# linomp/INF560-approximate-pattern-matching

Hardware: AMD Instinct MI355X
Metric: window-DP-cells/sec (higher is better)
Workload: dtype u32

## Files before the change

inf560-approximate-pattern-matching_amd/csrc/apm_device.h:

```cpp
#ifndef APM_DEVICE_H
#define APM_DEVICE_H

#include "apm_internal.h"
#include "apm_core.h"

__device__ __forceinline__ uint32_t apm_wave_count(bool pred) {
    return (uint32_t)__builtin_popcountll(__builtin_amdgcn_ballot_w64(pred));
}

__device__ __forceinline__ int apm_min3(int a, int b, int c) { return min(min(a, b), c); }

typedef unsigned int u32x4 __attribute__((ext_vector_type(4)));
typedef unsigned short u16x2 __attribute__((ext_vector_type(2)));
__device__ __forceinline__ u16x2 apm_as_u16x2(uint32_t v) { return __builtin_bit_cast(u16x2, v); }

__device__ __forceinline__ void apm_stage_image(uint4 *dst, const uint4 *src, int n16, int tid, int threads) {
    for (int i = tid; i < n16; i += 4 * threads) {
        const int i1 = i + threads, i2 = i + 2 * threads, i3 = i + 3 * threads;
        const uint4 v0 = src[i];
        const uint4 v1 = src[i1 < n16 ? i1 : i];
        const uint4 v2 = src[i2 < n16 ? i2 : i];
        const uint4 v3 = src[i3 < n16 ? i3 : i];
        dst[i] = v0;
        if (i1 < n16) dst[i1] = v1;
        if (i2 < n16) dst[i2] = v2;
        if (i3 < n16) dst[i3] = v3;
    }
}

template <int N>
__device__ __forceinline__ void apm_lds_dwords(const uint8_t *base, int off, uint32_t (&out)[N]) {
    const uint32_t *a = reinterpret_cast<const uint32_t *>(base) + (off >> 2);
    const uint32_t sh = (uint32_t)off & 3u;
    uint32_t w[N + 1];
#pragma unroll
    for (int i = 0; i <= N; ++i) w[i] = a[i];
#pragma unroll
    for (int i = 0; i < N; ++i) out[i] = __builtin_amdgcn_alignbyte(w[i + 1], w[i], sh);
}

template <int BAND, typename Text>
__device__ __forceinline__ bool apm_banded_verify(const Text &tx, const uint8_t *pb, int poff, int m, int k) {
    const uint8_t *p = pb + poff;
    if constexpr (BAND == 0 && Text::kBlocks) {
        int mism = 0;
        for (int xb = 0; xb < m; xb += 16) {
            uint32_t Tb[4], Pb[4];
            tx.load16_at(xb, Tb);
            apm_lds_dwords<4>(pb, poff + xb, Pb);
#pragma unroll
            for (int i = 0; i < 4; ++i) {
                const int valid = m - xb - 4 * i;
                const uint32_t mask = valid >= 4 ? 0xffffffffu : (valid <= 0 ? 0u : ((1u << (8 * valid)) - 1u));
                const uint32_t x = (Tb[i] ^ Pb[i]) & mask;
                mism += __builtin_popcount((x | ((x & 0x7f7f7f7fu) + 0x7f7f7f7fu)) & 0x80808080u);
            }
            if (mism > k) return false;
        }
        return true;
    } else if constexpr (BAND == 0) {
        int mism = 0;
        for (int x = 0; x < m; ++x) {
            mism += (tx.byte(x) != (int)p[x]) ? 1 : 0;
            if (mism > k) return false;
        }
        return true;
    } else {
        constexpr int NB = 2 * BAND + 1;
        constexpr int INF = 1 << 20;
        int e[NB];
#pragma unroll
        for (int i = 0; i < NB; ++i) e[i] = (i >= BAND) ? (i - BAND) : INF;
        int x0 = 1;
        if (m >= 16 && tx.can16(m)) {
            uint32_t T[4], P[5];
            tx.load16(T);
            apm_lds_dwords<5>(pb, poff, P);
#pragma unroll
            for (int x = 1; x <= 16; ++x) {
                const int tc = (int)((T[(x - 1) >> 2] >> (8 * ((x - 1) & 3))) & 0xffu);
                int up = INF, best = INF;
#pragma unroll
                for (int i = 0; i < NB; ++i) {
                    const int y = x + i - BAND;
                    int nv;
                    if (y < 1) {
                        nv = (y == 0) ? x : INF;
                    } else if (y > 16 && y > m) {
                        nv = INF;
                    } else {
                        const int pc = (int)((P[(y - 1) >> 2] >> (8 * ((y - 1) & 3))) & 0xffu);
                        const int diag = e[i] + ((pc != tc) ? 1 : 0);
                        const int left = (i + 1 < NB) ? e[i + 1] + 1 : INF;
                        nv = apm_min3(diag, left, up + 1);
                    }
                    e[i] = nv;
                    up = nv;
                    best = min(best, nv);
                }
                if ((x & 3) == 0 && best > k) return false;
            }
            x0 = 17;
            if constexpr (Text::kBlocks) {
                for (int xb = 17; xb <= m; xb += 16) {
                    uint32_t Tb[4], Pb[6];
                    tx.load16_at(xb - 1, Tb);
                    apm_lds_dwords<6>(pb, poff + xb - 1 - BAND, Pb);
#pragma unroll
                    for (int xi = 0; xi < 16; ++xi) {
                        const int x = xb + xi;
                        const int tc = (int)((Tb[xi >> 2] >> (8 * (xi & 3))) & 0xffu);
                        int up = INF, best = INF;
                        if (x <= m) {
#pragma unroll
                            for (int i = 0; i < NB; ++i) {
                                const int y = x + i - BAND;
                                int nv = INF;
                                if (y <= m) {
                                    const int pc = (int)((Pb[(xi + i) >> 2] >> (8 * ((xi + i) & 3))) & 0xffu);
                                    const int diag = e[i] + ((pc != tc) ? 1 : 0);
                                    const int left = (i + 1 < NB) ? e[i + 1] + 1 : INF;
                                    nv = apm_min3(diag, left, up + 1);
                                }
                                e[i] = nv;
                                up = nv;
                                best = min(best, nv);
                            }
                            if ((xi & 3) == 3 && best > k) return false;
                        }
                    }
                }
                return e[BAND] <= k;
            }
        }
        for (int x = x0; x <= m; ++x) {
            const int tc = tx.byte(x - 1);
            int up = INF;
            int best = INF;
#pragma unroll
            for (int i = 0; i < NB; ++i) {
                const int y = x + i - BAND;
                int nv;
                if (y < 1) {
                    nv = (y == 0) ? x : INF;
                } else if (y > m) {
                    nv = INF;
                } else {
                    const int diag = e[i] + (((int)p[y - 1] != tc) ? 1 : 0);
                    const int left = (i + 1 < NB) ? e[i + 1] + 1 : INF;
                    nv = apm_min3(diag, left, up + 1);
                }
                e[i] = nv;
                up = nv;
                best = min(best, nv);
            }
            if (best > k) return false;
        }
        return e[BAND] <= k;
    }
}

__device__ __forceinline__ uint32_t apm_bswap(uint32_t v) { return __builtin_bswap32(v); }

__device__ __forceinline__ void apm_push_pos(const ApmPosSink &ps, int64_t j_rel) {
    const unsigned long long idx = atomicAdd(ps.count, 1ull);
    if (idx < ps.cap) ps.out[idx] = ps.text_off + (unsigned long long)j_rel;
}

#ifdef APM_REC
__device__ __forceinline__ void apm_rec_store(const ApmPosSink &ps, unsigned long long idx, uint32_t pattern, int64_t j_rel) {
    if (idx < ps.cap) {
        const unsigned long long pos = ps.text_off + (unsigned long long)j_rel;
        reinterpret_cast<uint4 *>(ps.out)[idx] = make_uint4((uint32_t)pos, (uint32_t)(pos >> 32), pattern, 0u);
    }
}
__device__ __forceinline__ void apm_rec_push(const ApmPosSink &ps, uint32_t pattern, int64_t j_rel) {
    apm_rec_store(ps, atomicAdd(ps.count, 1ull), pattern, j_rel);
}
__device__ __forceinline__ void apm_rec_push_wave(const ApmPosSink &ps, bool hit, uint32_t pattern, int64_t j_rel) {
    const unsigned long long mask = __builtin_amdgcn_ballot_w64(hit);
    if (mask == 0ull) return;
    const uint32_t rank = __builtin_amdgcn_mbcnt_hi((uint32_t)(mask >> 32), __builtin_amdgcn_mbcnt_lo((uint32_t)mask, 0u));
    unsigned long long base = 0ull;
    if (hit && rank == 0u) base = atomicAdd(ps.count, (unsigned long long)__builtin_popcountll(mask));
    const int leader = __builtin_ctzll(mask);
    const uint32_t blo = (uint32_t)__builtin_amdgcn_readlane((int)(uint32_t)base, leader);
    const uint32_t bhi = (uint32_t)__builtin_amdgcn_readlane((int)(uint32_t)(base >> 32), leader);
    if (hit) apm_rec_store(ps, (((unsigned long long)bhi << 32) | blo) + rank, pattern, j_rel);
}
#define APM_SINK_LANE(ps, hit, pattern, j) apm_rec_push_wave((ps), (hit), (pattern), (j))
#else
#define APM_SINK_LANE(ps, hit, pattern, j) do { if ((ps).out && (hit)) apm_push_pos((ps), (j)); } while (0)
#endif


__device__ __forceinline__ void apm_tail_body(const ApmTailArgs &a, int pat_slot, uint4 *s_eq, int tid) {
    const ApmPatDesc d = a.pats[pat_slot];
    const int m = (int)d.m;
    const uint8_t *pat = a.bytes + d.byte_off;
    uint32_t *eqw = reinterpret_cast<uint32_t *>(s_eq);
    uint8_t *s_txt = reinterpret_cast<uint8_t *>(s_eq + 256);
    for (int i = tid; i < 1024; i += 128) eqw[i] = 0u;
    const int64_t first_trunc = max(a.jb, a.nrel - m + 1);
    const int64_t t0 = a.nrel - 128 > 0 ? a.nrel - 128 : 0;
    if (tid < 128) s_txt[tid] = (t0 + tid < a.nrel) ? a.text[t0 + tid] : (uint8_t)0;
    __syncthreads();
    if (tid < m) atomicOr(&eqw[(int)pat[tid] * 4 + (tid >> 5)], 1u << (tid & 31));
    __syncthreads();
    if (tid < 128) {
        const int64_t j = first_trunc + tid;
        const bool valid = j < a.je;
        const int size = valid ? (int)(a.nrel - j) : 0;
        const int lo = valid ? (int)(j - t0) : 0;
        uint32_t pv[4], mv[4];
        bp_init<4>(pv, mv);
        for (int x = 0; x < m - 1; ++x) {
            if (x < size) {
                const uint4 v = s_eq[s_txt[lo + x]];
                const uint32_t eq[4] = {v.x, v.y, v.z, v.w};
                bp_step<4>(pv, mv, eq);
            }
        }
        const bool hit = valid && bp_distance<4>(pv, mv, size, size) <= a.k;
        APM_SINK_LANE(a.pos, hit, d.index, j);
        const uint32_t cnt = apm_wave_count(hit);
        if ((tid & 63) == 0 && cnt) atomicAdd(&a.counts[d.index], (unsigned long long)cnt);
    }
}


__device__ __forceinline__ uint4 apm_load16_guarded(const uint8_t *text, int64_t pos, int64_t avail) {
    if (pos >= 0 && pos + 16 <= avail) return *reinterpret_cast<const uint4 *>(text + pos);
    uint32_t w[4] = {0u, 0u, 0u, 0u};
#pragma unroll
    for (int b = 0; b < 16; ++b) {
        const int64_t q = pos + b;
        if (q >= 0 && q < avail) w[b >> 2] |= (uint32_t)text[q] << (8 * (b & 3));
    }
    return make_uint4(w[0], w[1], w[2], w[3]);
}

#endif
```

inf560-approximate-pattern-matching_amd/csrc/apm_rec.h:

```cpp
#ifndef APM_REC_H
#define APM_REC_H
#ifdef APM_REC
#define apm_bitpar_kernel apm_bitpar_kernel_rec
#define apm_bitpar_xwide_kernel apm_bitpar_xwide_kernel_rec
#define apm_bitlong_kernel apm_bitlong_kernel_rec
#define apm_wavefront_kernel apm_wavefront_kernel_rec
#define apm_generic_kernel apm_generic_kernel_rec
#define apm_nfa_kernel apm_nfa_kernel_rec
#define apm_tail_kernel apm_tail_kernel_rec
#define apm_tail_wide_kernel apm_tail_wide_kernel_rec
#define apm_tail_xwide_kernel apm_tail_xwide_kernel_rec
#define apm_filter_kernel apm_filter_kernel_rec
#define apm_stream_kernel apm_stream_kernel_rec
#define apm_sieve2_kernel apm_sieve2_kernel_rec
#define apm_sieve2cf_kernel apm_sieve2cf_kernel_rec
#define apm_sieve2cfdp_kernel apm_sieve2cfdp_kernel_rec
#define apm_sieve2cfdg_kernel apm_sieve2cfdg_kernel_rec
#define apm_sieve8_kernel apm_sieve8_kernel_rec
#define apm_verify_kernel apm_verify_kernel_rec
#define apm_fused_kernel apm_fused_kernel_rec
#define apm_launch_bitpar apm_launch_bitpar_rec
#define apm_launch_bitpar_wide apm_launch_bitpar_wide_rec
#define apm_launch_bitpar_xwide apm_launch_bitpar_xwide_rec
#define apm_launch_bitlong apm_launch_bitlong_rec
#define apm_launch_wavefront apm_launch_wavefront_rec
#define apm_launch_generic apm_launch_generic_rec
#define apm_launch_nfa apm_launch_nfa_rec
#define apm_launch_tail apm_launch_tail_rec
#define apm_launch_tail_wide apm_launch_tail_wide_rec
#define apm_launch_tail_xwide apm_launch_tail_xwide_rec
#define apm_launch_filter apm_launch_filter_rec
#define apm_launch_stream apm_launch_stream_rec
#define apm_launch_sieve2 apm_launch_sieve2_rec
#define apm_launch_verify apm_launch_verify_rec
#define apm_launch_fused apm_launch_fused_rec
#define apm_bitpar_lds_bytes apm_bitpar_lds_bytes_rec
#define apm_bitlong_lds_bytes apm_bitlong_lds_bytes_rec
#define apm_wavefront_lds_bytes apm_wavefront_lds_bytes_rec
#define apm_nfa_lds_bytes apm_nfa_lds_bytes_rec
#define apm_filter_lds_bytes apm_filter_lds_bytes_rec
#define apm_filter_blocks_per_cu apm_filter_blocks_per_cu_rec
#define apm_filter_fn_b0 apm_filter_fn_b0_rec
#define apm_filter_fn_b1 apm_filter_fn_b1_rec
#define apm_filter_fn_b2 apm_filter_fn_b2_rec
#define apm_filter_fn_b2_dma apm_filter_fn_b2_dma_rec
#define apm_filter_fn_b3 apm_filter_fn_b3_rec
#define apm_stream_blocks_per_cu apm_stream_blocks_per_cu_rec
#define apm_sieve2cf_geometry apm_sieve2cf_geometry_rec
#define apm_sieve2cfdg_fn apm_sieve2cfdg_fn_rec
#define apm_sieve2cf_blocks apm_sieve2cf_blocks_rec
#define apm_verify_geometry apm_verify_geometry_rec
#define apm_fused_lds_bytes apm_fused_lds_bytes_rec
#define apm_fused_geometry apm_fused_geometry_rec
#endif
#endif
```

inf560-approximate-pattern-matching_amd/csrc/apm_scan.hip:

```cpp
#include "apm_state.h"
#include "apm_core.h"

#include <algorithm>
#include <cstdlib>
#include <cstring>

__global__ void apm_popcount_kernel(const uint32_t *w, unsigned long long n, unsigned long long *sum) {
    unsigned long long acc = 0;
    for (unsigned long long i = (unsigned long long)blockIdx.x * blockDim.x + threadIdx.x; i < n; i += (unsigned long long)gridDim.x * blockDim.x)
        acc += (unsigned long long)__popc(w[i]);
    for (int d = 32; d; d >>= 1) acc += __shfl_down(acc, d, 64);
    if ((threadIdx.x & 63) == 0 && acc) atomicAdd(sum, acc);
}

__global__ void apm_popcount_listed_kernel(const uint32_t *w, const uint32_t *blist, const uint32_t *n_listed, const uint32_t *clist_cnt, int regions, unsigned long long *sum) {
    unsigned long long acc = 0;
    const unsigned long long n = (unsigned long long)*n_listed * 64ull, t0 = (unsigned long long)blockIdx.x * blockDim.x + threadIdx.x;
    for (unsigned long long i = t0; i < n; i += (unsigned long long)gridDim.x * blockDim.x)
        acc += (unsigned long long)__popc(w[(unsigned long long)blist[i >> 6] * 64ull + (i & 63ull)]);
    for (unsigned long long i = t0; i < (unsigned long long)regions; i += (unsigned long long)gridDim.x * blockDim.x) acc += clist_cnt[i];
    for (int d = 32; d; d >>= 1) acc += __shfl_down(acc, d, 64);
    if ((threadIdx.x & 63) == 0 && acc) atomicAdd(sum, acc);
}

__global__ void apm_add_const_kernel(unsigned long long *counts, const int *idx, int n, unsigned long long v) {
    const int i = (int)(blockIdx.x * blockDim.x + threadIdx.x);
    if (i < n) atomicAdd(&counts[idx[i]], v);
}

__global__ void apm_rec_const_kernel(uint4 *out, unsigned long long *count, unsigned long long cap, const int *idx, int n,
                                     unsigned long long ob, unsigned long long oe) {
    const unsigned long long span = oe - ob, total = span * (unsigned long long)n;
    __shared__ unsigned long long s_base;
    const unsigned long long first = (unsigned long long)blockIdx.x * blockDim.x;
    for (unsigned long long b0 = first; b0 < total; b0 += (unsigned long long)gridDim.x * blockDim.x) {
        const unsigned long long here = total - b0 < blockDim.x ? total - b0 : blockDim.x;
        __syncthreads();
        if (threadIdx.x == 0) s_base = atomicAdd(count, here);
        __syncthreads();
        const unsigned long long i = b0 + threadIdx.x, at = s_base + threadIdx.x;
        if (i < total && at < cap) {
            const unsigned long long pos = ob + i % span;
            out[at] = make_uint4((uint32_t)pos, (uint32_t)(pos >> 32), (uint32_t)idx[i / span], 0u);
        }
    }
}

int note_launch(apm_ctx *ctx, DeviceState &ds, const char *label) {
    ds.launches++;
    if (!ctx->timing_on || ds.n_stamps >= DeviceState::MAX_STAMPS) return APM_OK;
    hipEvent_t &e = ds.ev_launch[ds.n_stamps];
    if (!e) HIP_TRY(ctx, hipEventCreate(&e));
    HIP_TRY(ctx, hipEventRecord(e, ds.stream));
    ds.launch_label[ds.n_stamps++] = label;
    return APM_OK;
}

int ensure_text(apm_ctx *ctx, DeviceState &ds, size_t bytes) {
    bytes = (bytes + 255) & ~(size_t)255;
    if (bytes <= ds.text_cap) return APM_OK;
    HIP_TRY(ctx, hipSetDevice(ds.dev));
    return grow_device_buffer(ctx, ds, (void **)&ds.d_text, &ds.text_cap, bytes, 1);
}

static int env_int(const char *name, int unset) { const char *v = getenv(name); return v ? atoi(v) : unset; }
static int env_1_to_64(const char *name, int unset) { return getenv(name) ? std::max(1, std::min(64, env_int(name, 0))) : unset; }
struct ScanEnv {
    int fused = env_int("APM_FUSED", -1);
    int blist = env_int("APM_SIEVE_BLIST", 1);
    int clist = env_int("APM_SIEVE_CLIST", 1);
    int clist_region_cap = env_1_to_64("APM_CLIST_REGION_CAP", 0);
    int clist_min_batch = env_1_to_64("APM_CLIST_MIN_BATCH", 8);
    int clist_pools = std::max(0, env_int("APM_CLIST_POOLS", 8));
    int cf_dp_diag = env_int("APM_CF_DP_DIAG", 1);
    int filter_dma = env_int("APM_FILTER_DMA", 1);
    int filter_stream = env_int("APM_FILTER_STREAM", 1);
#ifdef APM_MEASURE
    int qcap_s1 = env_int("APM_QCAP_S1", 0);
    int bpc_cap = env_int("APM_BPC_CAP", 0);
#endif
};
static const ScanEnv &scan_env() {
    static const ScanEnv env;
    return env;
}

struct ShardGeom {
    const uint8_t *text;
    int64_t jb, je;
    int64_t nrel;
    int64_t avail;
    int64_t avail_pad;
    int band;
    ApmPosSink sink;
    unsigned long long *counts;
    bool rec_on;
    bool aligned() const { return (reinterpret_cast<uintptr_t>(text) & 15u) == 0; }
};
#define APM_PICK(g, fn) ((g).rec_on ? fn##_rec : fn)

template <typename Args> static void set_common(Args &a, const apm_ctx *ctx, const ShardGeom &g, int64_t je) {
    a.text = g.text;
    a.jb = g.jb;
    a.je = je;
    a.nrel = g.nrel;
    a.counts = g.counts;
    a.k = ctx->k;
    a.pos = g.sink;
}

static int64_t aligned_tile0(const ShardGeom &g, int front = 0) {
    return g.jb - (int64_t)((reinterpret_cast<uintptr_t>(g.text) + (uintptr_t)g.jb - (uintptr_t)front) & 15u);
}

static bool has_tail_windows(const GenericGroup &grp, const ShardGeom &g) {
    return !grp.descs.empty() && g.nrel - (int64_t)grp.m_max + 1 < g.je;
}

struct ShortTails {
    ApmTailArgs args;
    int n = 0;
    bool pending = false;
    template <typename Args> void ride_with(Args &a) {
        if (!pending) return;
        a.n_tail = n;
        a.tail = args;
        pending = false;
    }
};

static int launch_generic_group(apm_ctx *ctx, DeviceState &ds, const ShardGeom &g, const GenericGroup &grp, const ApmPatDesc *d_descs, int mode) {
    if (grp.descs.empty() || g.je <= g.jb) return APM_OK;
    int64_t span = g.je - g.jb;
    if (mode == 1) span = std::min<int64_t>(span, grp.m_max);
    const size_t col = (size_t)grp.m_max + 1;
    const size_t budget = (size_t)1 << 30;
    const size_t per_launch = std::min<size_t>(grp.descs.size(), 65535);
    int64_t nbx = (span + APM_BLOCK - 1) / APM_BLOCK;
    const int64_t cap = std::max<int64_t>(1, (int64_t)(budget / (col * 2 * APM_BLOCK * per_launch)));
    nbx = std::max<int64_t>(1, std::min<int64_t>(std::min<int64_t>(nbx, cap), 4096));
    const size_t need = col * 2 * APM_BLOCK * (size_t)nbx * per_launch;
    const int rc = grow_device_buffer(ctx, ds, (void **)&ds.d_scratch, &ds.scratch_bytes, need, 1);
    if (rc) return rc;
    ApmGenericArgs a{};
    set_common(a, ctx, g, g.je);
    a.avail = g.avail;
    a.bytes = ds.d_allpat;
    a.mode = mode;
    a.col_stride = (int)col;
    a.scratch = ds.d_scratch;
    for (size_t first = 0; first < grp.descs.size(); first += per_launch) {
        a.pats = d_descs + first;
        APM_LAUNCH(ctx, ds, "generic", APM_PICK(g, apm_launch_generic)(a, (int)nbx, (int)std::min(per_launch, grp.descs.size() - first), ds.stream));
    }
    return APM_OK;
}

struct SieveRange {
    int64_t p_lo, p_hi;
    int64_t n_mask_blocks = 0;
    const uint32_t *blist_ctr = nullptr;
    int clist_regions = 0;
    uint32_t clist_region_cap = 0;
    int clist_pools = 0;
    uint32_t clist_pool_cap = 0;
    const uint32_t *cpool_cnt = nullptr;
    int64_t nchunks() const { return (p_hi - p_lo + 1023) / 1024; }
};
constexpr int kClistPerBlock = 32;
constexpr int kClistMaxRegions = 4096;

static ApmSieve2Args sieve_args(const SievePlan &S, const ShardGeom &g, const SieveRange &r, const uint32_t *d_bitmap) {
    ApmSieve2Args sv{};
    sv.text = g.text;
    sv.avail_pad = g.avail_pad;
    sv.tile0 = r.p_lo;
    sv.nchunks = r.nchunks();
    sv.bitmap = reinterpret_cast<const uint4 *>(d_bitmap);
    sv.code_shift = S.code_shift;
    sv.stride = S.stride;
    return sv;
}

static ApmVerifyArgs verify_args(const apm_ctx *ctx, const VerifyLaunch &V, const DevVerify &D, const ShardGeom &g, int64_t je_v) {
    const SievePlan &S = ctx->plan.sieve;
    ApmVerifyArgs va{};
    set_common(va, ctx, g, je_v);
    va.avail = g.avail;
    va.avail_pad = g.avail_pad;
    va.image = reinterpret_cast<const uint4 *>(D.d_image);
    va.image_len = (int)V.image.size();
    va.o_prefix = V.o_prefix;
    va.o_r2s = V.o_r2s;
    va.o_slots = V.o_slots;
    va.o_kext = V.o_kext;
    va.o_pat = V.o_pat;
    va.o_masks = V.o_masks;
    va.o_kinfo = V.o_kinfo;
    va.o_pinfo = V.o_pinfo;
    va.o_rc = V.o_rc;
    va.kinfo = D.d_kinfo;
    va.pinfo = reinterpret_cast<const uint2 *>(D.d_pinfo);
    va.kpart = D.d_kpart;
    va.pats = D.d_descs;
    va.n_pats = (int)V.descs.size();
    va.nk = (int)V.kinfo.size();
    va.band = g.band;
    va.code_shift = S.code_shift;
    va.stride = S.stride;
    return va;
}

static int run_fused(apm_ctx *ctx, DeviceState &ds, const ShardGeom &g, const SieveRange &r, ShortTails &tails, bool *ran) {
    const SievePlan &S = ctx->plan.sieve;
    bool fused_ok = scan_env().fused < 0 ? S.stride == 8 : scan_env().fused != 0;
    std::vector<ApmFusedArgs> fargs;
    std::vector<size_t> fa_index;
    for (size_t v = 0; fused_ok && v < S.launches.size(); ++v) {
        const VerifyLaunch &V = S.launches[v];
        DevVerify &D = ds.verify[v];
        ApmFusedArgs fa{};
        fa.s = sieve_args(S, g, r, ds.d_sieve_bmp);
        fa.v = verify_args(ctx, V, D, g, std::min<int64_t>(g.je, g.nrel - V.m_min + 1));
#ifdef APM_MEASURE
        if (!ds.d_stats) HIP_TRY(ctx, hipMalloc((void **)&ds.d_stats, APM_STATS_BYTES));
        fa.v.stats = ds.d_stats;
#endif
        if (!D.fused_threads) {
            D.fused_blocks_per_cu = apm_fused_geometry(fa, &D.fused_threads);
            if (D.fused_blocks_per_cu < 1) D.fused_threads = -1;
        }
        if (D.fused_threads < 64) fused_ok = false;
        if (fa.v.je > g.jb) { fargs.push_back(fa); fa_index.push_back(v); }
    }
    if (!fused_ok) return APM_OK;
    for (ApmFusedArgs &fa : fargs) {
        tails.ride_with(fa.s);
        const DevVerify &D = ds.verify[fa_index[&fa - fargs.data()]];
#ifdef APM_MEASURE
        HIP_TRY(ctx, hipMemsetAsync(ds.d_stats, 0, APM_STATS_BYTES, ds.stream));
#endif
        fa.v.work = ds.d_work;
        APM_LAUNCH(ctx, ds, "fused", APM_PICK(g, apm_launch_fused)(fa, D.fused_threads, ds.n_cu * D.fused_blocks_per_cu, &ds.work_epoch, ds.stream));
    }
    *ran = true;
    return APM_OK;
}

static int sieve_pass(apm_ctx *ctx, DeviceState &ds, const ShardGeom &g, SieveRange &r, ShortTails &tails, int v) {
    const SievePlan &S = ctx->plan.sieve;
    ApmSieve2PoolArgs sv{};
    static_cast<ApmSieve2Args &>(sv) = sieve_args(S, g, r, v < 0 ? ds.d_sieve_bmp : ds.verify[(size_t)v].d_bmp18);
    sv.masks = ds.d_masks;
    if (v >= 0) {
        const VerifyLaunch &V = S.launches[(size_t)v];
        const DevVerify &D = ds.verify[(size_t)v];
        sv.cf_image = reinterpret_cast<const uint4 *>(D.d_cf);
        sv.cf_len = (int)V.cf_image.size();
        sv.cf_o_rrec = V.cf_o_rrec;
        sv.cf_o_lrec = V.cf_o_lrec;
        sv.cf_threads = D.cf_threads;
        sv.cf_blocks_per_cu = D.cf_blocks_per_cu;
        sv.cf_o_dp = V.cf_o_dp;
        sv.cf_dp_k = ctx->k;
        sv.cf_dp_cols = V.cf_dp_cols;
    }
    if (v < 0 || tails.n <= 512) tails.ride_with(sv);
    const bool use_blist = scan_env().blist && sv.cf_image != nullptr;
    r.blist_ctr = nullptr;
    if (use_blist) {
        sv.blist = ds.d_blist;
        sv.blist_ctr = APM_BLIST_CTR(ds.d_work, ds.sieve_epoch & 1);
        sv.blist_ctr_next = APM_BLIST_CTR(ds.d_work, (ds.sieve_epoch + 1) & 1);
        r.blist_ctr = sv.blist_ctr;
    }
    r.clist_regions = 0;
    if (use_blist && scan_env().clist) {
        const size_t want = (size_t)r.n_mask_blocks * (size_t)kClistPerBlock + (size_t)kClistMaxRegions * 64;
        const int grc = grow_device_buffer(ctx, ds, (void **)&ds.d_clist, &ds.clist_cap, want, 4);
        if (grc) return grc;
        if (!ds.d_clist_cnt) HIP_TRY(ctx, hipMalloc((void **)&ds.d_clist_cnt, (size_t)kClistMaxRegions * 4));
        const int regions = apm_sieve2cf_blocks(sv, ds.n_cu);
        if (regions >= 1 && regions <= kClistMaxRegions) {
            r.clist_regions = regions;
            r.clist_region_cap = scan_env().clist_region_cap ? (uint32_t)scan_env().clist_region_cap
                                                             : (uint32_t)std::max<int64_t>(64, r.n_mask_blocks * kClistPerBlock / regions);
            sv.clist = ds.d_clist;
            sv.clist_cnt = ds.d_clist_cnt;
            sv.clist_cap = r.clist_region_cap;
        }
    }
    r.clist_pools = 0;
    if (r.clist_regions && scan_env().clist_pools > 0 && apm_cf_dp_form(sv.cf_o_dp > 0, sv.cf_dp_k, scan_env().cf_dp_diag != 0) == 2) {
        const int pools = std::min(scan_env().clist_pools, r.clist_regions);
        r.clist_pool_cap = (uint32_t)((r.clist_regions + pools - 1) / pools) * r.clist_region_cap;
        const int grc = grow_device_buffer(ctx, ds, (void **)&ds.d_cpool, &ds.cpool_cap, (size_t)pools * r.clist_pool_cap, 4);
        if (grc) return grc;
        if (!ds.d_cpool_cnt) {
            HIP_TRY(ctx, hipMalloc((void **)&ds.d_cpool_cnt, (size_t)2 * kClistMaxRegions * 4));
            HIP_TRY(ctx, hipMemsetAsync(ds.d_cpool_cnt, 0, (size_t)2 * kClistMaxRegions * 4, ds.stream));
        }
        sv.cpool = ds.d_cpool;
        sv.cpool_cnt = ds.d_cpool_cnt + (size_t)(ds.pool_epoch & 1) * kClistMaxRegions;
        sv.cpool_cnt_next = ds.d_cpool_cnt + (size_t)((ds.pool_epoch + 1) & 1) * kClistMaxRegions;
        sv.cpool_cap = r.clist_pool_cap;
        sv.cpool_n = pools;
        sv.cpool_next_n = ds.pool_dirty[(ds.pool_epoch + 1) & 1];
        r.cpool_cnt = sv.cpool_cnt;
    }
    ds.last_clist_regions = r.clist_regions;
    ds.last_blist_ctr = r.blist_ctr;
    ds.last_clist_pools = 0;
    HIP_TRY(ctx, APM_PICK(g, apm_launch_sieve2)(sv, ds.n_cu, ds.stream, scan_env().cf_dp_diag != 0, &ds.last_sieve_waves, &ds.last_cf_dp_form, &r.clist_pools));
    ds.last_clist_pools = r.clist_pools;
    if (use_blist) ++ds.sieve_epoch;
    if (r.clist_pools) {
        ds.pool_dirty[ds.pool_epoch & 1] = r.clist_pools;
        ds.pool_dirty[(ds.pool_epoch + 1) & 1] = 0;
        ++ds.pool_epoch;
    }
    return note_launch(ctx, ds, "sieve");
}

static int verify_pass(apm_ctx *ctx, DeviceState &ds, const ShardGeom &g, const SieveRange &r, size_t v, int64_t je_v) {
    DevVerify &D = ds.verify[v];
    ApmVerifyArgs va = verify_args(ctx, ctx->plan.sieve.launches[v], D, g, je_v);
    va.masks = ds.d_masks;
    if (r.blist_ctr) {
        va.blist = ds.d_blist;
        va.blist_ctr = r.blist_ctr;
    }
    if (r.clist_pools) {
        va.clist = ds.d_cpool;
        va.clist_cnt = r.cpool_cnt;
        va.clist_cap = r.clist_pool_cap;
        va.clist_regions = r.clist_pools;
        va.clist_min_batch = scan_env().clist_min_batch;
    } else if (r.clist_regions) {
        va.clist = ds.d_clist;
        va.clist_cnt = ds.d_clist_cnt;
        va.clist_cap = r.clist_region_cap;
        va.clist_regions = r.clist_regions;
        va.clist_min_batch = scan_env().clist_min_batch;
    }
    va.tile0 = r.p_lo;
    va.n_mask_blocks = r.n_mask_blocks;
#ifdef APM_MEASURE
    if (!ds.d_stats) HIP_TRY(ctx, hipMalloc((void **)&ds.d_stats, APM_STATS_BYTES));
    HIP_TRY(ctx, hipMemsetAsync(ds.d_stats, 0, APM_STATS_BYTES, ds.stream));
    va.stats = ds.d_stats;
#endif
    va.work = ds.d_work;
    if (!D.blocks_per_cu) D.blocks_per_cu = apm_verify_geometry(va, &D.threads);
    APM_LAUNCH(ctx, ds, "verify", APM_PICK(g, apm_launch_verify)(va, D.threads, ds.n_cu * D.blocks_per_cu, &ds.work_epoch, ds.stream));
    return APM_OK;
}

static int run_sieve_verify(apm_ctx *ctx, DeviceState &ds, const ShardGeom &g, SieveRange &r, ShortTails &tails) {
    const SievePlan &S = ctx->plan.sieve;
    r.n_mask_blocks = (r.nchunks() + 3) / 4;
    int rc = grow_device_buffer(ctx, ds, (void **)&ds.d_masks, &ds.masks_cap, (size_t)r.n_mask_blocks * 64 + 64, 4);
    if (rc) return rc;
    rc = grow_device_buffer(ctx, ds, (void **)&ds.d_blist, &ds.blist_cap, (size_t)r.n_mask_blocks + 64, 4);
    if (rc) return rc;
    ds.last_mask_blocks = r.n_mask_blocks;
    bool per_launch = S.per_launch_sieve;
    for (size_t v = 0; per_launch && v < S.launches.size(); ++v) {
        const VerifyLaunch &V = S.launches[v];
        DevVerify &D = ds.verify[v];
        if (!D.cf_threads) {
            D.cf_blocks_per_cu = apm_sieve2cf_geometry((int)V.cf_image.size(), apm_cf_dp_form(V.cf_o_dp > 0, ctx->k, scan_env().cf_dp_diag != 0), &D.cf_threads);
            if (D.cf_blocks_per_cu < 1) D.cf_threads = -1;
        }
        if (D.cf_threads < 64) per_launch = false;
    }
    bool any_pass = false;
    for (size_t v = 0; v < S.launches.size(); ++v) {
        const int64_t je_v = std::min<int64_t>(g.je, g.nrel - S.launches[v].m_min + 1);
        if (je_v <= g.jb) continue;
        if (per_launch || !any_pass) {
            rc = sieve_pass(ctx, ds, g, r, tails, per_launch ? (int)v : -1);
            if (rc) return rc;
            any_pass = true;
        }
        rc = verify_pass(ctx, ds, g, r, v, je_v);
        if (rc) return rc;
    }
    return APM_OK;
}

static int run_sieve_pipeline(apm_ctx *ctx, DeviceState &ds, const ShardGeom &g, ShortTails &tails, bool *fused_run, bool *sieve_run) {
    const SievePlan &S = ctx->plan.sieve;
    if (!S.on || !g.aligned()) return APM_OK;
    SieveRange r;
    r.p_lo = std::max<int64_t>(0, g.jb - g.band) & ~(int64_t)15;
    r.p_hi = std::min<int64_t>(g.avail, g.je + S.m_max + g.band);
    if (!(r.p_hi > r.p_lo && g.avail_pad >= 16 && g.avail_pad <= APM_SIEVE_MAX_BYTES)) return APM_OK;
    if (!ds.d_work) {
        HIP_TRY(ctx, hipMalloc((void **)&ds.d_work, APM_WORK_BYTES));
        HIP_TRY(ctx, hipMemsetAsync(ds.d_work, 0, APM_WORK_BYTES, ds.stream));
        ds.work_epoch = 0;
        ds.sieve_epoch = 0;
    }
    int rc = run_fused(ctx, ds, g, r, tails, fused_run);
    if (rc || *fused_run) return rc;
    rc = run_sieve_verify(ctx, ds, g, r, tails);
    if (rc) return rc;
    *sieve_run = true;
    return APM_OK;
}

static int launch_banded(apm_ctx *ctx, DeviceState &ds, const ShardGeom &g, const TiledLaunch &L, DevTiled &D, int64_t je_l, ShortTails &tails) {
    const ScanEnv &env = scan_env();
    ApmFilterArgs f{};
    set_common(f, ctx, g, je_l);
    f.avail = g.avail;
    f.avail_pad = g.avail_pad;
    f.band = g.band;
    f.front = f.band > 0 ? 16 : 0;
    f.tile0 = aligned_tile0(g, f.front);
    f.pats = D.d_descs;
    f.image = reinterpret_cast<const uint4 *>(D.d_image);
    f.image_len = (int)L.image.size();
    f.o_tab = L.o_tab;
    f.o_kid = L.o_kid;
    f.o_ovf = L.o_ovf;
    f.o_kinfo = L.o_kinfo;
    f.o_pinfo = L.o_pinfo;
    f.o_next = L.o_next;
    f.o_poff = L.o_poff;
    f.o_bmp = L.o_bmp;
    f.o_pat = L.o_pat;
    f.o_kext = L.o_kext;
    f.code_shift = L.code_shift;
    f.nk = (int)L.keys.size();
    f.nb = L.nb;
    f.lg_nb = L.lg_nb;
    f.n_ovf = (int)(L.ovf.size() / 2);
    f.qcap = L.qcap;
#ifdef APM_MEASURE
    if (L.stride == 1 && env.qcap_s1 >= 64 && env.qcap_s1 <= 8192) f.qcap = env.qcap_s1;
#endif
    f.key_len = L.key_len;
    f.stride = L.stride;
    f.n_cu = ds.n_cu;
    f.n_pats = (int)L.descs.size();
    f.tile_w = L.tile;
    f.tile_len = APM_FILTER_POS;
    f.ntiles = (je_l - f.tile0 + L.tile - 1) / L.tile;
    const bool can_load16 = g.aligned() && f.avail_pad >= 16;
    f.use_dma = (env.filter_dma && can_load16) ? 1 : 0;
    const double hit_rate = (double)L.keys.size() / (double)(1ull << (2 * std::min(L.key_len, 8)));
    const bool stream_ok = L.stride > 1 || (f.band <= 1 && (env.filter_stream == 2 || (env.filter_stream != 3 && hit_rate < 1.0 / 200.0)));
    if (env.filter_stream && stream_ok && can_load16) {
        const int64_t p_lo = std::max<int64_t>(0, g.jb - f.band) & ~(int64_t)15;
        const int64_t p_hi = std::min<int64_t>(g.avail, je_l + L.m_max + f.band);
        f.tile0 = p_lo;
        f.ntiles = p_hi > p_lo ? (p_hi - p_lo + 1023) / 1024 : 0;
        if (!D.blocks_per_cu[2]) D.blocks_per_cu[2] = apm_stream_blocks_per_cu(f);
        tails.ride_with(f);
        APM_LAUNCH(ctx, ds, "stream", APM_PICK(g, apm_launch_stream)(f, ds.n_cu * D.blocks_per_cu[2], ds.stream));
        return APM_OK;
    }
    if (!D.blocks_per_cu[f.use_dma])
        D.blocks_per_cu[f.use_dma] = apm_filter_blocks_per_cu(f.band, f.key_len, f.stride, f.use_dma, apm_filter_lds_bytes(f));
    tails.ride_with(f);
    int bpc = D.blocks_per_cu[f.use_dma];
#ifdef APM_MEASURE
    if (env.bpc_cap > 0) bpc = std::min(env.bpc_cap, bpc);
#endif
    APM_LAUNCH(ctx, ds, "tile", APM_PICK(g, apm_launch_filter)(f, ds.n_cu * bpc, ds.stream));
    return APM_OK;
}

static int launch_nfa(apm_ctx *ctx, DeviceState &ds, const ShardGeom &g, const TiledLaunch &L, const DevTiled &D, int64_t je_l) {
    ApmNfaArgs na{};
    set_common(na, ctx, g, je_l);
    na.avail = g.avail;
    na.tile0 = aligned_tile0(g);
    na.pats = D.d_descs;
    na.classes = D.d_bytes;
    na.cls_len = (int)L.bytes.size();
    memcpy(na.class_bytes, L.lut, 16);
    na.n_classes = L.nb;
    na.n_pats = (int)L.descs.size();
    APM_LAUNCH(ctx, ds, "nfa", APM_PICK(g, apm_launch_nfa)(na, ds.stream));
    return APM_OK;
}

static int launch_full_dp(apm_ctx *ctx, DeviceState &ds, const ShardGeom &g, const TiledLaunch &L, const DevTiled &D, int64_t je_l) {
    const bool per_wave = L.kind == APM_KERNEL_BITPAR && L.m_max > 1024;
    ApmScanArgs a{};
    set_common(a, ctx, g, per_wave ? g.je : je_l);
    a.avail = g.avail;
    a.tile0 = aligned_tile0(g);
    a.pats = D.d_descs;
    a.tables = D.d_tables;
    a.lut = D.d_lut;
    a.n_pats = per_wave ? 1 : (int)L.descs.size();
    a.table_words = (int)L.tables.size();
    if (per_wave) {
        APM_LAUNCH(ctx, ds, "bitpar", APM_PICK(g, apm_launch_bitlong)(a, L.m_max, ds.stream));
        return APM_OK;
    }
    a.bytes = D.d_bytes;
    a.tile = L.tile;
    a.halo = L.m_max - 1;
    a.bytes_len = (int)L.bytes.size();
    if (L.kind == APM_KERNEL_BITPAR) APM_LAUNCH(ctx, ds, "bitpar", APM_PICK(g, apm_launch_bitpar)(a, ds.stream));
    else APM_LAUNCH(ctx, ds, "wavefront", APM_PICK(g, apm_launch_wavefront)(a, ds.stream));
    return APM_OK;
}

static int run_tiled_launches(apm_ctx *ctx, DeviceState &ds, const ShardGeom &g, ShortTails &tails, bool sieved) {
    for (size_t t = 0; t < ctx->plan.tiled.size(); ++t) {
        const TiledLaunch &L = ctx->plan.tiled[t];
        const bool per_wave = L.kind == APM_KERNEL_BITPAR && L.m_max > 1024;
        const int64_t je_l = std::min<int64_t>(g.je, g.nrel - L.m_min + 1);
        if (!per_wave && je_l <= g.jb) continue;
        int rc;
        if (L.kind == APM_KERNEL_BANDED) {
            if (sieved && L.sieved) continue;
            rc = launch_banded(ctx, ds, g, L, ds.tiled[t], je_l, tails);
        } else if (L.kind == APM_KERNEL_NFA) {
            rc = launch_nfa(ctx, ds, g, L, ds.tiled[t], je_l);
        } else {
            rc = launch_full_dp(ctx, ds, g, L, ds.tiled[t], je_l);
        }
        if (rc) return rc;
    }
    return APM_OK;
}

static int run_tails_and_trivial(apm_ctx *ctx, DeviceState &ds, const ShardGeom &g, ShortTails &tails, uint64_t ob, uint64_t oe) {
    const ApmPlan &plan = ctx->plan;
    typedef hipError_t (*TailLauncher)(const ApmTailArgs &, int, hipStream_t);
    const struct { bool due; const GenericGroup &grp; const ApmPatDesc *d_descs; TailLauncher count, rec; } classes[3] = {
        {tails.pending, plan.stails, ds.d_stail_descs, apm_launch_tail, apm_launch_tail_rec},
        {has_tail_windows(plan.wtails, g), plan.wtails, ds.d_wtail_descs, apm_launch_tail_wide, apm_launch_tail_wide_rec},
        {has_tail_windows(plan.xtails, g), plan.xtails, ds.d_xtail_descs, apm_launch_tail_xwide, apm_launch_tail_xwide_rec},
    };
    for (const auto &c : classes) {
        if (!c.due) continue;
        ApmTailArgs ta = tails.args;
        ta.pats = c.d_descs;
        APM_LAUNCH(ctx, ds, "tail", (g.rec_on ? c.rec : c.count)(ta, (int)c.grp.descs.size(), ds.stream));
    }
    if (!plan.trivial.empty()) {
        const int nt = (int)plan.trivial.size();
        hipLaunchKernelGGL(apm_add_const_kernel, dim3((unsigned)((nt + 255) / 256)), dim3(256), 0, ds.stream, g.counts,
                           ds.d_trivial, nt, (unsigned long long)(oe - ob));
        if (g.rec_on) {
            const unsigned long long total = (unsigned long long)(oe - ob) * (unsigned long long)nt;
            const unsigned nb = (unsigned)std::min<unsigned long long>((total + 255) / 256, 4096);
            hipLaunchKernelGGL(apm_rec_const_kernel, dim3(nb), dim3(256), 0, ds.stream, reinterpret_cast<uint4 *>(g.sink.out), g.sink.count,
                               g.sink.cap, ds.d_trivial, nt, (unsigned long long)ob, (unsigned long long)oe);
        }
    }
    HIP_TRY(ctx, hipGetLastError());
    return APM_OK;
}

static int scan_shard_one(apm_ctx *ctx, DeviceState &ds, const ShardText &sh, uint64_t own_begin, uint64_t own_end,
                          unsigned long long *d_counts, const ApmPosSink *rec) {
    const uint8_t *d_text = sh.text;
    const uint64_t text_off = sh.text_off, text_len = sh.text_len, n_total = sh.n_total;
    const ApmPlan &plan = ctx->plan;
    const uint64_t k = (uint64_t)ctx->k;
    const uint64_t limit = n_total > k ? n_total - k : 0;
    const uint64_t ob = own_begin, oe = std::min(own_end, limit);
    if (oe <= ob) return APM_OK;
    if (text_off > ob) return fail(ctx, APM_ERR_INVALID, "shard text starts after own_begin");
    const uint64_t m_max = (uint64_t)std::max(plan.m_max, 1);
    const uint64_t need_end = std::min<uint64_t>(n_total, oe + m_max - 1);
    if (text_off + text_len < need_end)
        return fail(ctx, APM_ERR_INVALID, "shard text too short: halo of m_max-1 = %llu bytes required",
                    (unsigned long long)(m_max - 1));
    HIP_TRY(ctx, hipSetDevice(ds.dev));
    ds.text_bytes += need_end - ob;

    ShardGeom g{};
    g.text = d_text;
    g.jb = (int64_t)(ob - text_off);
    g.je = (int64_t)(oe - text_off);
    g.nrel = (int64_t)(n_total - text_off);
    g.avail = (int64_t)text_len;
    g.avail_pad = g.avail + (int64_t)((16u - ((reinterpret_cast<uintptr_t>(d_text) + (uintptr_t)g.avail) & 15u)) & 15u);
    g.band = ctx->k / 2;
    g.counts = d_counts;
    g.rec_on = rec != nullptr;
    if (rec) {
        g.sink = *rec;
        g.sink.text_off = text_off;
    } else if (ctx->find_active) {
        g.sink.out = ds.d_pos_out;
        g.sink.count = ds.d_pos_count;
        g.sink.cap = ds.pos_cap;
        g.sink.text_off = text_off;
    }
    ShortTails tails;
    set_common(tails.args, ctx, g, g.je);
    tails.args.pats = ds.d_stail_descs;
    tails.args.bytes = ds.d_allpat;
    tails.n = (int)plan.stails.descs.size();
    tails.pending = has_tail_windows(plan.stails, g);

    if (ctx->timing_on) HIP_TRY(ctx, hipEventRecord(ds.ev_mstart, ds.stream));
    bool fused_run = false, sieve_run = false;
    int rc = run_sieve_pipeline(ctx, ds, g, tails, &fused_run, &sieve_run);
    if (rc) return rc;
    rc = run_tiled_launches(ctx, ds, g, tails, fused_run || sieve_run);
    if (rc) return rc;
    ds.last_fused = fused_run;
    if (!sieve_run) { ds.last_mask_blocks = 0; ds.last_clist_regions = 0; ds.last_clist_pools = 0; ds.last_sieve_waves = 0; ds.last_cf_dp_form = 0; }
    rc = launch_generic_group(ctx, ds, g, plan.longs, ds.d_long_descs, 2);
    if (rc) return rc;
    if (ctx->timing_on) HIP_TRY(ctx, hipEventRecord(ds.ev_mstop, ds.stream));
    if (has_tail_windows(plan.tails, g)) {
        rc = launch_generic_group(ctx, ds, g, plan.tails, ds.d_tail_descs, 1);
        if (rc) return rc;
    }
    return run_tails_and_trivial(ctx, ds, g, tails, ob, oe);
}

int scan_shard(apm_ctx *ctx, DeviceState &ds, const ShardText &sh, uint64_t own_begin, uint64_t own_end, unsigned long long *d_counts,
               const ApmPosSink *rec) {
    const uint8_t *d_text = sh.text;
    uint64_t text_off = sh.text_off, text_len = sh.text_len;
    const uint64_t n_total = sh.n_total;
    const bool sieve_on = ctx->plan.sieve.on;
    const uint64_t lim32 = (uint64_t)APM_SIEVE_MAX_BYTES - 4096;
    const uint64_t mis = (uint64_t)(reinterpret_cast<uintptr_t>(d_text) & 15u);
    if (sieve_on && mis != 0 && text_off >= mis && text_len > 0) {
        d_text -= mis;
        text_off -= mis;
        text_len += mis;
    }
    if (!sieve_on || text_len < lim32 || (reinterpret_cast<uintptr_t>(d_text) & 15u) != 0 || own_begin < text_off)
        return scan_shard_one(ctx, ds, ShardText{d_text, text_off, text_len, n_total}, own_begin, own_end, d_counts, rec);
    const uint64_t k = (uint64_t)ctx->k;
    const uint64_t oe = std::min(own_end, n_total > k ? n_total - k : 0);
    const uint64_t m_max = (uint64_t)std::max(ctx->plan.m_max, 1), step = (uint64_t)3 << 30;
    for (uint64_t b = own_begin; b < oe;) {
        const uint64_t e = std::min(oe, b + step);
        const uint64_t sb = text_off + ((b - text_off) & ~(uint64_t)15);
        const uint64_t se = std::min(text_off + text_len, e + m_max + 31);
        const int rc = scan_shard_one(ctx, ds, ShardText{d_text + (sb - text_off), sb, se - sb, n_total}, b, e, d_counts, rec);
        if (rc) return rc;
        b = e;
    }
    return APM_OK;
}

int sieve_candidates(apm_ctx *ctx, DeviceState &ds, double *value) {
    *value = 0;
    if (!ds.d_masks || ds.last_mask_blocks <= 0) return APM_OK;
    HIP_TRY(ctx, hipSetDevice(ds.dev));
    if (!ds.d_stats) HIP_TRY(ctx, hipMalloc((void **)&ds.d_stats, APM_STATS_BYTES));
    unsigned long long *d_sum = ds.d_stats + 7;
    HIP_TRY(ctx, hipMemsetAsync(d_sum, 0, 8, ds.stream));
    if (ds.last_clist_regions)
        hipLaunchKernelGGL(apm_popcount_listed_kernel, dim3(1024), dim3(256), 0, ds.stream, ds.d_masks, ds.d_blist, ds.last_blist_ctr, ds.d_clist_cnt, ds.last_clist_regions, d_sum);
    else
        hipLaunchKernelGGL(apm_popcount_kernel, dim3(1024), dim3(256), 0, ds.stream, ds.d_masks, (unsigned long long)ds.last_mask_blocks * 64ull, d_sum);
    unsigned long long h = 0;
    HIP_TRY(ctx, hipMemcpyAsync(&h, d_sum, 8, hipMemcpyDeviceToHost, ds.stream));
    HIP_TRY(ctx, hipStreamSynchronize(ds.stream));
    *value = (double)h;
    return APM_OK;
}
```

inf560-approximate-pattern-matching_amd/csrc/apm_sieve.h:

```cpp
#ifndef APM_SIEVE_H
#define APM_SIEVE_H

#include "apm_internal.h"

struct ApmSieve2Args {
    const uint8_t *text;
    int64_t avail_pad;
    int64_t tile0;
    int64_t nchunks;
    const uint4 *bitmap;
    int code_shift;
    int stride;
    uint32_t *masks;
    uint32_t *blist;
    uint32_t *blist_ctr, *blist_ctr_next;
    uint32_t *clist;
    uint32_t *clist_cnt;
    uint32_t clist_cap;
    int n_main_blocks;
    int n_tail;
    ApmTailArgs tail;
    const uint4 *cf_image;
    int cf_len, cf_o_rrec, cf_o_lrec;
    int cf_o_dp, cf_dp_k, cf_dp_cols;
    int cf_threads, cf_blocks_per_cu;
#ifdef APM_MEASURE
    int skip_mask;
#endif
};
struct ApmSieve2PoolArgs : ApmSieve2Args {
    uint32_t *cpool;
    uint32_t *cpool_cnt, *cpool_cnt_next;
    uint32_t cpool_cap;
    int cpool_n;
    int cpool_next_n;
};
#define APM_SIEVE_MAX_BYTES (((int64_t)1 << 32) - ((int64_t)64 << 20))
#define APM_CF_WAVE_BYTES 1552
#define APM_CF_DP_PEND_BYTES 128
#define APM_CF_DP_COLS 30
#define APM_CF_DP_SLOTS 7
static inline int apm_cf_dp_form(bool dp, int k, bool diag_on) { return !dp ? 0 : (diag_on && k <= 3 ? 2 : 1); }
const void *apm_sieve2cfdg_fn();
int apm_sieve2cf_geometry(int cf_len, int dp_form, int *threads);
int apm_sieve2cf_blocks(const ApmSieve2Args &a, int n_cu);

struct ApmVerifyArgs {
    const uint8_t *text;
    int64_t avail;
    int64_t avail_pad;
    int64_t jb, je, nrel;
    const uint4 *image;
    int image_len, o_prefix, o_r2s, o_slots, o_kext, o_pat;
    int o_masks;
    int o_rc;
    int o_kinfo, o_pinfo;
    const uint32_t *kinfo;
    const uint2 *pinfo;
    const uint32_t *kpart;
    const ApmPatDesc *pats;
    unsigned long long *counts;
    int n_pats, nk, k, band, code_shift;
    int stride;
    const uint32_t *masks;
    const uint32_t *blist;
    const uint32_t *blist_ctr;
    const uint32_t *clist;
    const uint32_t *clist_cnt;
    uint32_t clist_cap;
    int clist_regions;
    int clist_min_batch;
    int64_t tile0;
    int64_t n_mask_blocks;
    int n_blocks;
    uint32_t *work;
    int work_epoch;
    int work_groups;
#ifdef APM_MEASURE
    int skip_mask;
    unsigned long long *stats;
#endif
    ApmPosSink pos;
};

struct ApmFusedArgs {
    ApmSieve2Args s;
    ApmVerifyArgs v;
};
#define APM_FUSED_MAX_THREADS 896
hipError_t apm_launch_fused(const ApmFusedArgs &a, int threads, int max_blocks, int *work_epoch, hipStream_t s);
size_t apm_fused_lds_bytes(const ApmFusedArgs &a, int threads);
int apm_fused_geometry(const ApmFusedArgs &a, int *threads);

#define APM_WORK_GROUPS 32
#define APM_WORK_STRIDE 64
#define APM_WORK_BYTES (2 * APM_WORK_GROUPS * APM_WORK_STRIDE * 4 + 2 * APM_WORK_STRIDE * 4)
#define APM_BLIST_CTR(work, set) ((work) + 2 * APM_WORK_GROUPS * APM_WORK_STRIDE + (set) * APM_WORK_STRIDE)
#define APM_STATS_WAVES 16384
#define APM_STATS_BYTES (64 + 16 * APM_STATS_WAVES)
hipError_t apm_launch_sieve2(const ApmSieve2PoolArgs &a, int n_cu, hipStream_t s, bool dp_diag, int *cf_waves, int *cf_dp_form, int *clist_pools);
hipError_t apm_launch_verify(const ApmVerifyArgs &a, int threads, int max_blocks, int *work_epoch, hipStream_t s);
int apm_verify_geometry(const ApmVerifyArgs &a, int *threads);
#ifndef APM_REC
hipError_t apm_launch_fused_rec(const ApmFusedArgs &a, int threads, int max_blocks, int *work_epoch, hipStream_t s);
hipError_t apm_launch_sieve2_rec(const ApmSieve2PoolArgs &a, int n_cu, hipStream_t s, bool dp_diag, int *cf_waves, int *cf_dp_form, int *clist_pools);
hipError_t apm_launch_verify_rec(const ApmVerifyArgs &a, int threads, int max_blocks, int *work_epoch, hipStream_t s);
#endif

#endif
```

inf560-approximate-pattern-matching_amd/csrc/apm_state.h:

```cpp
#ifndef APM_STATE_H
#define APM_STATE_H

#include "../../include/apm.h"
#include "apm_plan.h"
#include "apm_sieve.h"
#include "apm_textnorm.h"
#include "apm_seqindex.h"

#include <string>
#include <vector>

struct DevVerify {
    uint32_t *d_bmp18 = nullptr;
    uint8_t *d_cf = nullptr;
    ApmPatDesc *d_descs = nullptr;
    uint8_t *d_image = nullptr;
    uint32_t *d_kinfo = nullptr;
    uint32_t *d_pinfo = nullptr;
    uint32_t *d_kpart = nullptr;
    int blocks_per_cu = 0, threads = 256;
    int fused_blocks_per_cu = 0, fused_threads = 0;
    int cf_threads = 0, cf_blocks_per_cu = 0;
};

struct DevTiled {
    ApmPatDesc *d_descs = nullptr;
    uint8_t *d_bytes = nullptr;
    uint32_t *d_tables = nullptr;
    uint8_t *d_lut = nullptr;
    uint8_t *d_image = nullptr;
    int blocks_per_cu[3] = {0, 0, 0};
};

struct DeviceState {
    int dev = -1;
    int n_cu = 256;
    hipStream_t stream = nullptr;
    hipStream_t own_stream = nullptr;
    uint8_t *d_allpat = nullptr;
    ApmPatDesc *d_tail_descs = nullptr;
    ApmPatDesc *d_stail_descs = nullptr;
    ApmPatDesc *d_wtail_descs = nullptr;
    ApmPatDesc *d_xtail_descs = nullptr;
    ApmPatDesc *d_long_descs = nullptr;
    int *d_trivial = nullptr;
    std::vector<DevTiled> tiled;
    unsigned long long *d_counts = nullptr;
    uint16_t *d_scratch = nullptr;
    size_t scratch_bytes = 0;
    unsigned long long *d_pos_out = nullptr;
    unsigned long long *d_pos_count = nullptr;
    unsigned long long pos_cap = 0;
    unsigned long long *d_rec = nullptr;
    size_t rec_cap = 0;
    unsigned long long *d_rec_n = nullptr;
    uint8_t *d_score_img = nullptr;
    uint2 *d_score_tab = nullptr;
    void *d_align_ws = nullptr;
    uint32_t align_rows = 0;
    uint32_t last_align_rows = 0;
    uint32_t *d_ops = nullptr;
    size_t ops_cap = 0;
    unsigned long long *d_rec2 = nullptr;
    size_t rec2_cap = 0;
    hipEvent_t ev_best[2] = {};
    bool best_timed = false;
    uint32_t occ_segment = 0;
    uint64_t occ_lanes = 0;
    uint32_t nearest_segment = 0;
    uint64_t nearest_lanes = 0;
    unsigned long long *d_nearest_keys = nullptr;
    size_t nearest_keys_cap = 0;
    uint8_t *d_text = nullptr;
    size_t text_cap = 0;
    uint8_t *d_raw = nullptr;
    size_t raw_cap = 0;
    uint32_t *d_tn_summary = nullptr;
    unsigned long long *d_tn_map = nullptr;
    unsigned long long *d_tn_total = nullptr;
    size_t tn_cap = 0;
    ApmTnSrc tn_src{};
    bool tn_valid = false;
    uint64_t tn_src_bytes = 0, tn_kept_bytes = 0;
    hipEvent_t ev_tn[4] = {};
    bool tn_timed = false, map_timed = false;
    uint32_t *d_sq_count = nullptr;
    unsigned long long *d_sq_prefix = nullptr;
    unsigned long long *d_sq_total = nullptr;
    size_t sq_cap = 0;
    uint64_t sq_n_seq = 0;
    bool tn_host = false;
    apm_seq *d_seq_table = nullptr;
    size_t seq_table_cap = 0;
    uint64_t seq_table_n = 0;
    uint8_t *d_loc_buf = nullptr;
    size_t loc_buf_cap = 0;
    hipEvent_t ev_sq[4] = {};
    bool sq_timed = false, locate_timed = false;
    hipEvent_t ev_stage[32] = {};
    uint32_t *d_sieve_bmp = nullptr;
    std::vector<DevVerify> verify;
    uint32_t *d_masks = nullptr;
    size_t masks_cap = 0;
    int64_t last_mask_blocks = 0;
    uint32_t *d_work = nullptr;
    int work_epoch = 0;
    uint32_t *d_blist = nullptr;
    size_t blist_cap = 0;
    int sieve_epoch = 0;
    uint32_t *d_clist = nullptr;
    uint32_t *d_clist_cnt = nullptr;
    size_t clist_cap = 0;
    int last_clist_regions = 0;
    const uint32_t *last_blist_ctr = nullptr;
    uint32_t *d_cpool = nullptr;
    uint32_t *d_cpool_cnt = nullptr;
    size_t cpool_cap = 0;
    int pool_epoch = 0;
    int pool_dirty[2] = {0, 0};
    int last_clist_pools = 0;
    unsigned long long *d_stats = nullptr;
    int last_sieve_waves = 0;
    int last_cf_dp_form = 0;
    bool last_fused = false;
    hipEvent_t ev_start = nullptr, ev_kstart = nullptr, ev_mstart = nullptr, ev_mstop = nullptr, ev_stop = nullptr;
    bool events_recorded = false;
    static constexpr int MAX_STAMPS = 32;
    hipEvent_t ev_launch[MAX_STAMPS] = {};
    const char *launch_label[MAX_STAMPS] = {};
    int n_stamps = 0;
    uint64_t text_bytes = 0;
    int launches = 0;
};

struct RcclApi {
    void *handle = nullptr;
    int (*CommInitAll)(void **, int, const int *) = nullptr;
    int (*CommDestroy)(void *) = nullptr;
    int (*AllReduce)(const void *, void *, size_t, int, int, void *, hipStream_t) = nullptr;
    int (*GroupStart)() = nullptr;
    int (*GroupEnd)() = nullptr;
    std::vector<void *> comms;
    bool ready = false;
};

struct apm_ctx {
    std::vector<DeviceState> devs;
    std::vector<PatternInfo> pats;
    ApmPlan plan;
    int k = 0;
    int kernel = APM_KERNEL_AUTO;
    bool patterns_set = false;
    bool timing_on = true;
    bool find_active = false;
    unsigned text_mode = 0;
    std::string err;
    apm_timing timing{};
    RcclApi rccl;
    bool multi = false;
    int partition = APM_PARTITION_TEXT;
    std::vector<apm_ctx *> children;
    std::vector<int> pat_first;
    static constexpr int N_STAGE = 32;
    static constexpr size_t STAGE_BYTES = (size_t)8 << 20;
    uint8_t *stage[N_STAGE] = {};
};

int fail(apm_ctx *ctx, int code, const char *fmt, ...);

#define HIP_TRY(ctx, expr)                                                                      \
    do {                                                                                        \
        hipError_t _e = (expr);                                                                 \
        if (_e != hipSuccess)                                                                   \
            return fail(ctx, APM_ERR_HIP, "%s failed: %s (%s:%d)", #expr, hipGetErrorString(_e), \
                        __FILE__, __LINE__);                                                    \
    } while (0)

int note_launch(apm_ctx *ctx, DeviceState &ds, const char *label);

#define APM_LAUNCH(ctx, ds, label, expr)                 \
    do {                                                 \
        HIP_TRY(ctx, expr);                              \
        const int _nrc = note_launch(ctx, ds, label);    \
        if (_nrc) return _nrc;                           \
    } while (0)

struct ShardText {
    const uint8_t *text;
    uint64_t text_off, text_len, n_total;
};

int scan_shard(apm_ctx *ctx, DeviceState &ds, const ShardText &sh, uint64_t own_begin, uint64_t own_end, unsigned long long *d_counts,
               const ApmPosSink *rec = nullptr);
int sieve_candidates(apm_ctx *ctx, DeviceState &ds, double *value);
int ensure_text(apm_ctx *ctx, DeviceState &ds, size_t bytes);

__attribute__((visibility("hidden"))) int grow_device_buffer(apm_ctx *ctx, DeviceState &ds, void **ptr, size_t *cap, size_t want, size_t elem_bytes,
                                                             int status = APM_ERR_HIP, const char *noun_fmt = nullptr, ...);

#endif
```

inf560-approximate-pattern-matching_amd/csrc/apm_stats.hip:

```cpp
#include "apm_runtime.h"
#include "apm_core.h"

#include <cstdlib>
#include <string>
#include <vector>

void account(apm_ctx *ctx, uint64_t n_total, uint64_t ob, uint64_t oe) {
    const uint64_t k = (uint64_t)ctx->k;
    const uint64_t limit = n_total > k ? n_total - k : 0;
    oe = std::min(oe, limit);
    if (oe <= ob) return;
    for (const auto &p : ctx->pats) {
        const uint64_t m = (uint64_t)p.m;
        const uint64_t full_end = n_total >= m ? std::min<uint64_t>(oe, n_total - m + 1) : 0;
        const uint64_t nfull = full_end > ob ? full_end - ob : 0;
        double cells = double(nfull) * double(m) * double(m);
        for (uint64_t j = std::max(ob, full_end); j < oe; ++j) {
            const double s = double(n_total - j);
            cells += s * s;
        }
        ctx->timing.windows += oe - ob;
        ctx->timing.cells_algorithmic += cells;
        if (p.kernel == APM_KERNEL_BANDED || p.kernel == APM_KERNEL_NFA)
            ctx->timing.cells_evaluated += double(oe - ob) * double(m) * double(2 * (ctx->k / 2) + 1);
        else if (p.kernel != KERNEL_TRIVIAL)
            ctx->timing.cells_evaluated += cells;
    }
}

void begin_call(apm_ctx *ctx) {
    ctx->timing = apm_timing{};
    ctx->timing.n_devices = (int)ctx->devs.size();
    for (auto &ds : ctx->devs) {
        ds.text_bytes = 0;
        ds.launches = 0;
        ds.n_stamps = 0;
        ds.events_recorded = false;
    }
}

int collect_event_times(apm_ctx *ctx) {
    double kmax = 0, mmax = 0, hmax = 0;
    uint64_t bytes = 0;
    int launches = 0;
    for (auto &ds : ctx->devs) {
        bytes += ds.text_bytes;
        launches += ds.launches;
        if (!ds.events_recorded) continue;
        HIP_TRY(ctx, hipSetDevice(ds.dev));
        HIP_TRY(ctx, hipEventSynchronize(ds.ev_stop));
        float h = 0, kk = 0, mm = 0;
        hipEventElapsedTime(&h, ds.ev_start, ds.ev_kstart);
        hipEventElapsedTime(&kk, ds.ev_kstart, ds.ev_stop);
        if (hipEventElapsedTime(&mm, ds.ev_mstart, ds.ev_mstop) != hipSuccess) mm = 0;
        hmax = std::max<double>(hmax, h);
        kmax = std::max<double>(kmax, kk);
        mmax = std::max<double>(mmax, mm);
    }
    ctx->timing.h2d_ms = hmax;
    ctx->timing.kernel_ms = kmax;
    ctx->timing.main_kernel_ms = mmax;
    ctx->timing.text_bytes = bytes;
    ctx->timing.n_launches = launches;
    return APM_OK;
}

extern "C" {

int apm_get_timing(const apm_ctx *cctx, apm_timing *out) {
    apm_ctx *ctx = const_cast<apm_ctx *>(cctx);
    if (!ctx || !out) return APM_ERR_INVALID;
    if (pattern_sharded(ctx)) { *out = ctx->timing; return APM_OK; }
    const int rc = collect_event_times(ctx);
    if (rc) return rc;
    *out = ctx->timing;
    return APM_OK;
}

int apm_get_launch_times(const apm_ctx *cctx, int max, double *ms, const char **labels) {
    apm_ctx *ctx = const_cast<apm_ctx *>(cctx);
    if (!ctx || max < 0 || (max > 0 && !ms)) return APM_ERR_INVALID;
    if (ctx->devs.empty()) return 0;
    DeviceState &ds = ctx->devs[0];
    if (!ds.events_recorded || ds.n_stamps == 0) return 0;
    HIP_TRY(ctx, hipSetDevice(ds.dev));
    HIP_TRY(ctx, hipEventSynchronize(ds.ev_launch[ds.n_stamps - 1]));
    const int n = std::min(max, ds.n_stamps);
    for (int i = 0; i < n; ++i) {
        float t = 0;
        if (hipEventElapsedTime(&t, i ? ds.ev_launch[i - 1] : ds.ev_mstart, ds.ev_launch[i]) != hipSuccess) t = 0;
        ms[i] = t;
        if (labels) labels[i] = ds.launch_label[i];
    }
    return n;
}

int apm_get_stat(const apm_ctx *cctx, const char *name, double *value) {
    apm_ctx *ctx = const_cast<apm_ctx *>(cctx);
    if (!ctx || !name || !value || ctx->devs.empty()) return APM_ERR_INVALID;
    DeviceState &ds = ctx->devs[0];
    const std::string n = name;
    const SievePlan &S = ctx->plan.sieve;
    static const DevVerify no_verify;
    const DevVerify &G0 = ds.verify.empty() ? no_verify : ds.verify[0];
    if (n == "sieve_on") { *value = S.on ? 1 : 0; return APM_OK; }
    if (n == "sieve_rate") { *value = S.rate; return APM_OK; }
    if (n == "sieve_fused") { *value = ds.last_fused ? 1 : 0; return APM_OK; }
    if (n == "sieve_cf") { *value = (S.on && S.per_launch_sieve && G0.cf_threads >= 64) ? (double)G0.cf_threads : 0.0; return APM_OK; }
    if (n == "sieve_weak_frac") { *value = S.weak_frac; return APM_OK; }
    if (n == "sieve_cf_dp_slots") { *value = S.per_launch_sieve ? (double)S.launches[0].cf_dp_slots : 0.0; return APM_OK; }
    if (n == "sieve_cf_dp_form") { *value = (double)ds.last_cf_dp_form; return APM_OK; }
    if (n == "sieve_cf_waves_per_cu") { *value = (S.per_launch_sieve && G0.cf_threads >= 64) ? (double)(G0.cf_threads / 64 * G0.cf_blocks_per_cu) : 0.0; return APM_OK; }
    if (n == "sieve_cf_bytes") { *value = S.per_launch_sieve ? (double)S.launches[0].cf_image.size() : 0.0; return APM_OK; }
    if (n == "sieve_stride") { *value = S.on ? (double)S.stride : 0.0; return APM_OK; }
    if (n == "sieve_clist") { *value = ds.last_clist_regions ? 1.0 : 0.0; return APM_OK; }
    if (n == "sieve_clist_pools") { *value = (double)ds.last_clist_pools; return APM_OK; }
    if (n == "sieve_waves") { *value = (double)ds.last_sieve_waves; return APM_OK; }
    if (n == "sieve_mask_bytes") {
        *value = (double)ds.last_mask_blocks * 256.0;
        if (ds.last_clist_regions && ds.last_mask_blocks > 0) {
            HIP_TRY(ctx, hipSetDevice(ds.dev));
            std::vector<uint32_t> cnt((size_t)ds.last_clist_regions);
            uint32_t listed = 0;
            HIP_TRY(ctx, hipMemcpyAsync(cnt.data(), ds.d_clist_cnt, cnt.size() * 4, hipMemcpyDeviceToHost, ds.stream));
            HIP_TRY(ctx, hipMemcpyAsync(&listed, ds.last_blist_ctr, 4, hipMemcpyDeviceToHost, ds.stream));
            HIP_TRY(ctx, hipStreamSynchronize(ds.stream));
            double entries = 0;
            for (uint32_t c : cnt) entries += (double)c;
            *value = 4.0 * entries + 256.0 * (double)listed;
        }
        return APM_OK;
    }
    if (n == "verify_launches") { *value = (double)S.launches.size(); return APM_OK; }
    if (n == "verify_image_bytes") { *value = S.launches.empty() ? 0.0 : (double)S.launches[0].image.size(); return APM_OK; }
    if (n == "verify_blocks_per_cu") {
        *value = S.launches.empty() ? 0.0 : (double)(ds.last_fused ? G0.fused_blocks_per_cu : G0.blocks_per_cu);
        return APM_OK;
    }
    if (n == "verify_threads") {
        *value = S.launches.empty() ? 0.0 : (double)(ds.last_fused ? G0.fused_threads : G0.threads);
        return APM_OK;
    }
    if (n == "sieve_candidates") return sieve_candidates(ctx, ds, value);
    if (n == "align_rows") { *value = (double)ds.last_align_rows; return APM_OK; }
    if (n == "norm_src_bytes") { *value = (double)ds.tn_src_bytes; return APM_OK; }
    if (n == "norm_kept_bytes") { *value = (double)ds.tn_kept_bytes; return APM_OK; }
    if (n == "seq_count") { *value = (double)ds.sq_n_seq; return APM_OK; }
    if (n == "seq_index_ms" || n == "locate_ms") {
        const int at = n == "seq_index_ms" ? 0 : 2;
        *value = 0.0;
        if (at == 0 ? ds.sq_timed : ds.locate_timed) {
            HIP_TRY(ctx, hipSetDevice(ds.dev));
            HIP_TRY(ctx, hipEventSynchronize(ds.ev_sq[at + 1]));
            float t = 0;
            HIP_TRY(ctx, hipEventElapsedTime(&t, ds.ev_sq[at], ds.ev_sq[at + 1]));
            *value = t;
        }
        return APM_OK;
    }
    if (n == "occ_segment") { *value = (double)ds.occ_segment; return APM_OK; }
    if (n == "occ_lanes") { *value = (double)ds.occ_lanes; return APM_OK; }
    if (n == "nearest_segment") { *value = (double)ds.nearest_segment; return APM_OK; }
    if (n == "nearest_lanes") { *value = (double)ds.nearest_lanes; return APM_OK; }
    if (n == "best_ms") {
        *value = 0.0;
        if (ds.best_timed) {
            HIP_TRY(ctx, hipSetDevice(ds.dev));
            HIP_TRY(ctx, hipEventSynchronize(ds.ev_best[1]));
            float t = 0;
            HIP_TRY(ctx, hipEventElapsedTime(&t, ds.ev_best[0], ds.ev_best[1]));
            *value = t;
        }
        return APM_OK;
    }
    if (n == "norm_ms" || n == "map_ms") {
        const int at = n == "norm_ms" ? 0 : 2;
        *value = 0.0;
        if (at == 0 ? ds.tn_timed : ds.map_timed) {
            HIP_TRY(ctx, hipSetDevice(ds.dev));
            HIP_TRY(ctx, hipEventSynchronize(ds.ev_tn[at + 1]));
            float t = 0;
            HIP_TRY(ctx, hipEventElapsedTime(&t, ds.ev_tn[at], ds.ev_tn[at + 1]));
            *value = t;
        }
        return APM_OK;
    }
#ifdef APM_MEASURE
    if (n.rfind("verify_", 0) == 0 && ds.d_stats) {
        HIP_TRY(ctx, hipSetDevice(ds.dev));
        HIP_TRY(ctx, hipStreamSynchronize(ds.stream));
        unsigned long long h[8] = {};
        HIP_TRY(ctx, hipMemcpy(h, ds.d_stats, 64, hipMemcpyDeviceToHost));
        if (n == "verify_survivors") { *value = (double)h[1]; return APM_OK; }
        if (n == "verify_dp_items") { *value = (double)h[2]; return APM_OK; }
        if (n == "verify_counted") { *value = (double)h[3]; return APM_OK; }
        if (n.rfind("verify_wave_", 0) == 0) {
            std::vector<unsigned long long> t(2 * APM_STATS_WAVES);
            HIP_TRY(ctx, hipMemcpy(t.data(), ds.d_stats + 8, t.size() * 8, hipMemcpyDeviceToHost));
            std::vector<double> st, en;
            unsigned long long t0 = ~0ull;
            for (size_t w = 0; w < APM_STATS_WAVES; ++w) if (t[2 * w + 1]) t0 = std::min(t0, t[2 * w]);
            for (size_t w = 0; w < APM_STATS_WAVES; ++w) if (t[2 * w + 1]) { st.push_back((double)(t[2 * w] - t0) * 0.01); en.push_back((double)(t[2 * w + 1] - t0) * 0.01); }
            if (n.rfind("verify_wave_grp", 0) == 0 || n.rfind("verify_wave_xcd", 0) == 0) {
                const bool by_xcd = n[12] == 'x';
                const int want = atoi(n.c_str() + 18);
                double lo = 1e30, hi = 0, sum = 0; long cnt = 0;
                for (size_t w = 0; w < APM_STATS_WAVES; ++w) {
                    if (!t[2 * w + 1]) continue;
                    const int key = by_xcd ? (int)((w / 4) % 8) : (int)((w ^ (w >> 5)) % APM_WORK_GROUPS);
                    if (key != want) continue;
                    const double e = (double)(t[2 * w + 1] - t0) * 0.01;
                    lo = std::min(lo, e); hi = std::max(hi, e); sum += e; ++cnt;
                }
                *value = n[15] == 'm' && n[16] == 'a' ? hi : (n[15] == 'm' && n[16] == 'i' ? lo : (cnt ? sum / cnt : 0));
                return APM_OK;
            }
            if (n.rfind("verify_wave_slow", 0) == 0) {
                const bool end = n.rfind("verify_wave_slowend", 0) == 0;
                const size_t want = (size_t)atoi(n.c_str() + (end ? 19 : 16));
                std::vector<std::pair<unsigned long long, size_t>> by_end;
                for (size_t w = 0; w < APM_STATS_WAVES; ++w) if (t[2 * w + 1]) by_end.push_back({t[2 * w + 1], w});
                std::sort(by_end.rbegin(), by_end.rend());
                if (want >= by_end.size()) { *value = -1; return APM_OK; }
                *value = end ? (double)(by_end[want].first - t0) * 0.01 : (double)by_end[want].second;
                return APM_OK;
            }
            if (en.empty()) { *value = 0; return APM_OK; }
            std::sort(st.begin(), st.end());
            std::sort(en.begin(), en.end());
            if (n == "verify_wave_count") { *value = (double)en.size(); return APM_OK; }
            if (n == "verify_wave_start_max") { *value = st.back(); return APM_OK; }
            if (n == "verify_wave_end_min") { *value = en.front(); return APM_OK; }
            if (n == "verify_wave_end_p10") { *value = en[en.size() / 10]; return APM_OK; }
            if (n == "verify_wave_end_p50") { *value = en[en.size() / 2]; return APM_OK; }
            if (n == "verify_wave_end_p90") { *value = en[en.size() * 9 / 10]; return APM_OK; }
            if (n == "verify_wave_end_max") { *value = en.back(); return APM_OK; }
        }
    }
#endif
    return fail(ctx, APM_ERR_INVALID, "unknown statistic '%s'", name);
}

}
```

inf560-approximate-pattern-matching_amd/csrc/apm_verify.hip:

```cpp
#include <algorithm>
#include "apm_wave.h"
#include "apm_sieve.h"
#include "apm_launch.h"

#ifndef APM_WORK_CH
#define APM_WORK_CH 8u
#endif
#ifndef APM_WORK_CH8
#define APM_WORK_CH8 8u
#endif
#ifndef APM_VERIFY_PIPE
#define APM_VERIFY_PIPE 2
#endif
#ifndef APM_FUSED_PIPE
#define APM_FUSED_PIPE 1
#endif
#ifndef APM_VERIFY_AHEAD
#define APM_VERIFY_AHEAD 2
#endif
#ifndef APM_FUSED_S_WAVES
#define APM_FUSED_S_WAVES 6
#endif
#ifndef APM_DEDUP_PREFETCH
#define APM_DEDUP_PREFETCH(band, sampled, fused) (!(fused) && !(sampled))
#endif
#ifndef APM_DEDUP_WIDE
#define APM_DEDUP_WIDE(band, sampled, fused) ((band) >= 1)
#endif

struct ApmBufText {
    __amdgpu_buffer_rsrc_t rs;
    uint32_t off;
    static constexpr bool kBlocks = true;
    __device__ __forceinline__ bool can16(int) const { return true; }
    __device__ __forceinline__ void load16(uint32_t (&T)[4]) const { load16_at(0, T); }
    __device__ __forceinline__ void load16_at(int x0, uint32_t (&T)[4]) const {
        const uint32_t a0 = (off + (uint32_t)x0) & ~3u, sh = (off + (uint32_t)x0) & 3u;
        const u32x4 lo = __builtin_amdgcn_raw_buffer_load_b128(rs, (int)a0, 0, 0);
        const uint32_t hi = __builtin_amdgcn_raw_buffer_load_b32(rs, (int)(a0 + 16u), 0, 0);
        T[0] = __builtin_amdgcn_alignbyte(lo.y, lo.x, sh);
        T[1] = __builtin_amdgcn_alignbyte(lo.z, lo.y, sh);
        T[2] = __builtin_amdgcn_alignbyte(lo.w, lo.z, sh);
        T[3] = __builtin_amdgcn_alignbyte(hi, lo.w, sh);
    }
    __device__ __forceinline__ int byte(int x) const { return (int)__builtin_amdgcn_raw_buffer_load_b8(rs, (int)(off + (uint32_t)x), 0, 0); }
};

struct ApmWin { uint32_t w[6]; };

template <int BAND>
struct ApmVerifyCore {
    static constexpr int NSH = 2 * BAND + 1;
    static constexpr bool PAIRS = BAND >= 1;
    const ApmVerifyArgs &a;
    __amdgpu_buffer_rsrc_t rs;
    uint32_t avail;
    const uint32_t *s_kext;
    const uint4 *s_masks;
    const uint8_t *s_pat;
    uint32_t *s_cnt;
    int lane;
    const uint32_t *s_kinfo;
    const uint2 *s_pinfo;

    __device__ __forceinline__ void load_global(uint32_t a0, ApmWin &o) const {
        const u32x4 lo = __builtin_amdgcn_raw_buffer_load_b128(rs, (int)a0, 0, 0);
        const v2u32 hi = __builtin_amdgcn_raw_buffer_load_b64(rs, (int)(a0 + 16u), 0, 0);
        o.w[0] = lo.x; o.w[1] = lo.y; o.w[2] = lo.z; o.w[3] = lo.w; o.w[4] = hi.x; o.w[5] = hi.y;
    }
    __device__ __forceinline__ int gbyte(uint32_t pos) const {
        return (int)__builtin_amdgcn_raw_buffer_load_b8(rs, (int)pos, 0, 0);
    }

    template <typename LoadWin>
    __device__ __forceinline__ bool stage1(uint32_t kid, uint32_t s, const ApmWin &win, LoadWin &&load_win) const {
        typedef unsigned long long u64;
        const uint32_t kx = s_kext[kid];
        const int at = (int)(kx & 0xffffu), len = (int)((kx >> 16) & 0xffu), n = (int)((kx >> 24) & 31u), side = (int)(kx >> 29);
        if ((u64)s + (u64)len > (u64)avail) return false;
        const uint32_t sh = s & 3u;
        uint32_t A[4], B[4];
#pragma unroll
        for (int i = 0; i < 4; ++i) A[i] = __builtin_amdgcn_alignbyte(win.w[i + 1], win.w[i], sh);
        apm_lds_dwords<4>(s_pat, at, B);
        const uint4 mk = s_masks[len < 16 ? len : 16];
        if ((((A[0] ^ B[0]) & mk.x) | ((A[1] ^ B[1]) & mk.y) | ((A[2] ^ B[2]) & mk.z) | ((A[3] ^ B[3]) & mk.w)) != 0u) return false;
        for (int x = 16; x < len; ++x)
            if (gbyte(s + (uint32_t)x) != (int)s_pat[at + x]) return false;
        if (!PAIRS || side == 0) return true;
        if (n == 31) {
            const uint32_t kp = a.kpart[kid];
            const int poff = (int)(s_pinfo[s_kinfo[kid] & 0xfffu].x & 0xffffu), ap = (int)(kp & 0xffffu), nn = (int)(kp >> 16), ap1 = ap + nn;
            const bool fwd = side == 1;
            auto T = [&](int i) { return fwd ? gbyte(s + (uint32_t)len + (uint32_t)i) : gbyte(s - 1u - (uint32_t)i); };
            auto P = [&](int i) { return fwd ? (int)s_pat[poff + ap + i] : (int)s_pat[poff + ap1 - 1 - i]; };
            int i = 0;
            while (i < nn && T(i) == P(i)) ++i;
            if (i >= nn - 1) return true;
            bool ok = true;
            for (int j = i + 1; j < nn && ok; ++j) ok = T(j) == P(j);
            if (ok) return true;
            ok = true;
            for (int j = i + 1; j < nn && ok; ++j) ok = T(j - 1) == P(j);
            if (ok) return true;
            ok = true;
            for (int j = i; j < nn && ok; ++j) ok = T(j + 1) == P(j);
            return ok;
        }
        uint32_t P[4], T[5];
        ApmWin tw;
        if (side == 1) {
            const uint32_t tp = s + (uint32_t)len;
            if (len == 0 || APM_SKIP(a, 1024)) tw = win;
            else load_win(tp & ~3u, tw);
            apm_lds_dwords<4>(s_pat, at + len, P);
#pragma unroll
            for (int i = 0; i < 5; ++i) T[i] = __builtin_amdgcn_alignbyte(tw.w[i + 1], tw.w[i], tp & 3u);
        } else {
            uint32_t Q[4], Wd[5];
            apm_lds_dwords<4>(s_pat, at - 16, Q);
            if (s >= 20u) {
                const uint32_t tp = s - 20u;
                if (APM_SKIP(a, 1024)) tw = win;
                else load_win(tp & ~3u, tw);
#pragma unroll
                for (int i = 0; i < 5; ++i) Wd[i] = __builtin_amdgcn_alignbyte(tw.w[i + 1], tw.w[i], tp & 3u);
            } else {
#pragma unroll
                for (int i = 0; i < 5; ++i) Wd[i] = 0u;
                for (int i = 20 - (int)s; i < 20; ++i) {
                    const uint32_t b = (uint32_t)gbyte(s - 20u + (uint32_t)i);
#pragma unroll
                    for (int d = 0; d < 5; ++d)
                        if ((i >> 2) == d) Wd[d] |= b << (8 * (i & 3));
                }
            }
#pragma unroll
            for (int z = 0; z < 4; ++z) P[z] = apm_bswap(Q[3 - z]);
#pragma unroll
            for (int z = 0; z < 5; ++z) T[z] = apm_bswap(Wd[4 - z]);
        }
        if (n >= 4) {
            auto nz4 = [](uint32_t x) { return apm_udot4((((x & 0x7f7f7f7fu) + 0x7f7f7f7fu) | x) >> 7 & 0x01010101u, 0x08040201u); };
            const uint32_t z0 = nz4(P[0] ^ T[0]);
            if (z0 & (z0 - 1u)) {
                const uint32_t i = (uint32_t)__builtin_ctz(z0);
                const uint32_t z1 = nz4(P[0] ^ (T[0] << 8));
                const uint32_t z2 = nz4(P[0] ^ __builtin_amdgcn_alignbyte(T[1], T[0], 1u));
                if (((z1 >> (i + 1u)) != 0u) && ((z2 >> i) != 0u)) return false;
            }
        }
        return apm_ext1_core16(P, T, n);
    }


    __device__ __forceinline__ bool dp_match(uint32_t kid, uint32_t s, int dl, uint32_t &wpat, uint32_t &wj, uint32_t &word) const {
        const uint32_t ki = s_kinfo[kid];
        const int kpat = (int)(ki & 0xfffu), koff = (int)((ki >> 12) & 0x1ffu), kunit = (int)((ki >> 21) & 7u);
        const uint2 pinf = s_pinfo[kpat];
        const int poff = (int)(pinf.x & 0xffffu), m = (int)(pinf.x >> 16);
        const int64_t je_p = min(a.je, a.nrel - m + 1);
        const int64_t j = (int64_t)s - koff - dl;
        if (j < a.jb || j >= je_p) return false;
        wpat = (uint32_t)kpat;
        wj = (uint32_t)j;
        word = (uint32_t)(kunit * NSH + dl + BAND);
#ifdef APM_MEASURE
        if (APM_SKIP(a, 256)) atomicAdd(&a.stats[2], 1ull);
#endif
        return apm_banded_verify<BAND>(ApmBufText{rs, (uint32_t)j}, s_pat, poff, m, a.k);
    }

    template <bool PREF>
    __device__ __forceinline__ bool nominates(uint32_t bpat, uint32_t bj, int idx) const {
        const uint32_t kid = s_pinfo[bpat].y + (uint32_t)(idx / NSH);
        const int dd = idx % NSH - BAND;
        const int64_t o = (int64_t)bj + (int)((s_kinfo[kid] >> 12) & 0x1ffu) + dd;
        if (o < 0) return false;
        ApmWin w2;
        load_global((uint32_t)o & ~3u, w2);
        if constexpr (PAIRS && PREF) {
            const uint32_t kx = s_kext[kid];
            const uint32_t len = (kx >> 16) & 0xffu, side = kx >> 29;
            const bool ask = side != 0u && ((kx >> 24) & 31u) != 31u && (side == 1u ? len != 0u : o >= 20);
            const uint32_t pa = ask ? (side == 1u ? (uint32_t)o + len : (uint32_t)o - 20u) & ~3u : 0xffffff00u;
            ApmWin wp;
            load_global(pa, wp);
            return stage1(kid, (uint32_t)o, w2, [&](uint32_t a0, ApmWin &o2) {
                if (a0 == pa) o2 = wp;
                else load_global(a0, o2);
            });
        }
        return stage1(kid, (uint32_t)o, w2, [&](uint32_t a0, ApmWin &o2) { load_global(a0, o2); });
    }

    template <bool WIDE, bool PREF>
    __device__ __forceinline__ void count_matches(bool hit, uint32_t wpat, uint32_t wj, uint32_t word) const {
        for (unsigned long long m2 = __builtin_amdgcn_ballot_w64(hit); m2; m2 &= m2 - 1ull) {
            const int src = __builtin_ctzll(m2);
            const uint32_t bpat = (uint32_t)__builtin_amdgcn_readlane((int)wpat, src), bj = (uint32_t)__builtin_amdgcn_readlane((int)wj, src);
            const uint32_t bord = (uint32_t)__builtin_amdgcn_readlane((int)word, src);
            if (hit && wpat == bpat && wj == bj && word > bord) hit = false;
        }
        unsigned long long hm = __builtin_amdgcn_ballot_w64(hit);
        if constexpr (WIDE) {
            if (!hm) return;
#ifdef APM_MEASURE
            if (APM_SKIP(a, 32)) return;
#endif
            const unsigned long long pm = __builtin_amdgcn_ballot_w64(hit && word != 0u);
            unsigned long long dup = 0ull;
            uint32_t total = 0;
            for (unsigned long long mm = pm; mm; mm &= mm - 1ull) total += (uint32_t)__builtin_amdgcn_readlane((int)word, __builtin_ctzll(mm));
            for (uint32_t base = 0; base < total; base += 64u) {
                const uint32_t t = base + (uint32_t)lane;
                uint32_t msrc = 0, mfirst = 0, run = 0;
                for (unsigned long long mm = pm; mm; mm &= mm - 1ull) {
                    const int src = __builtin_ctzll(mm);
                    if (t >= run) { msrc = (uint32_t)src; mfirst = run; }
                    run += (uint32_t)__builtin_amdgcn_readlane((int)word, src);
                }
                const uint32_t bpat = (uint32_t)__builtin_amdgcn_ds_bpermute((int)(msrc << 2), (int)wpat);
                const uint32_t bj = (uint32_t)__builtin_amdgcn_ds_bpermute((int)(msrc << 2), (int)wj);
                const bool earlier = t < total && nominates<PREF>(bpat, bj, (int)(t - mfirst));
                unsigned long long em = __builtin_amdgcn_ballot_w64(earlier);
                while (em) {
                    const int l = __builtin_ctzll(em);
                    const uint32_t sl = (uint32_t)__builtin_amdgcn_readlane((int)msrc, l);
                    dup |= 1ull << sl;
                    em &= ~__builtin_amdgcn_ballot_w64(msrc == sl);
                }
            }
            const bool counts = hit && !((dup >> lane) & 1ull);
            if (counts) atomicAdd(&s_cnt[wpat], 1u);
#ifdef APM_REC
            apm_rec_push_wave(a.pos, counts, counts ? a.pats[wpat].index : 0u, (int64_t)wj);
#endif
#ifdef APM_MEASURE
            if (APM_SKIP(a, 256) && counts) atomicAdd(&a.stats[3], 1ull);
#endif
            return;
        }
        while (hm) {
            const int src = __builtin_ctzll(hm);
            hm &= hm - 1ull;
            const uint32_t bpat = (uint32_t)__builtin_amdgcn_readlane((int)wpat, src), bj = (uint32_t)__builtin_amdgcn_readlane((int)wj, src);
            const int n_before = __builtin_amdgcn_readlane((int)word, src);
#ifdef APM_MEASURE
            if (APM_SKIP(a, 32)) continue;
#endif
            const bool earlier = lane < n_before && nominates<false>(bpat, bj, lane);
            if (!__builtin_amdgcn_ballot_w64(earlier) && lane == 0) {
                atomicAdd(&s_cnt[bpat], 1u);
#ifdef APM_REC
                apm_rec_push(a.pos, a.pats[bpat].index, (int64_t)bj);
#endif
#ifdef APM_MEASURE
                if (APM_SKIP(a, 256)) atomicAdd(&a.stats[3], 1ull);
#endif
            }
        }
    }

};

__host__ __device__ constexpr int apm_verify_scap(int band) { return ((64 + 2 * band) / (2 * band + 1) + 63 + 7) & ~7; }

template <int BAND, int THREADS_T, bool SAMPLED, bool FUSED>
__device__ __forceinline__ void apm_verify_body(const ApmVerifyArgs &a, const ApmSieve2Args *sv, uint8_t *smem) {
    const int THREADS = THREADS_T ? THREADS_T : (int)blockDim.x;
    const int tid = threadIdx.x, lane = tid & 63;
    const int wv = __builtin_amdgcn_readfirstlane(tid >> 6);
    constexpr int NSH = 2 * BAND + 1;
    constexpr uint32_t FLUSH_AT = (64 + NSH - 1) / NSH;
    (void)FLUSH_AT;
    constexpr int SCAP = apm_verify_scap(BAND);
    uint8_t *s_img = smem + ((FUSED && !SAMPLED) ? 32768 : 0);
    const uint32_t *s_bmp = reinterpret_cast<const uint32_t *>(s_img);
    const uint16_t *s_prefix = reinterpret_cast<const uint16_t *>(s_img + a.o_prefix);
    const uint16_t *s_r2s = reinterpret_cast<const uint16_t *>(s_img + a.o_r2s);
    const uint16_t *s_slots = reinterpret_cast<const uint16_t *>(s_img + a.o_slots);
    const ApmKeyList keys{s_bmp, s_prefix, s_r2s, s_slots};
    const uint32_t *s_kext = reinterpret_cast<const uint32_t *>(s_img + a.o_kext);
    const uint8_t *s_pat = s_img + a.o_pat;
    const uint4 *s_masks = reinterpret_cast<const uint4 *>(s_img + a.o_masks);
    uint32_t *s_cnt = reinterpret_cast<uint32_t *>(s_img + a.image_len);
    uint2 *s_surv = reinterpret_cast<uint2 *>(s_cnt + ((a.n_pats + 3) & ~3)) + wv * SCAP;
    uint32_t *s_q = reinterpret_cast<uint32_t *>(reinterpret_cast<uint2 *>(s_cnt + ((a.n_pats + 3) & ~3)) + (THREADS / 64) * SCAP) + wv * 128;

    const uint32_t my_wave = blockIdx.x * (uint32_t)(THREADS / 64) + (uint32_t)wv;
    const uint32_t n_listed = (!FUSED && a.blist != nullptr) ? *a.blist_ctr : 0xffffffffu;
    bool cl_on = false;
    uint32_t cl_r = 0, cl_rstep = 0, cl_b = 0, cl_bstep = 1, cl_n = 0, cl_bs = 64;
    if constexpr (!FUSED && !SAMPLED) {
        if (a.clist) {
            const uint32_t R = (uint32_t)a.clist_regions, Wv = (uint32_t)gridDim.x * (uint32_t)(THREADS / 64);
            if (Wv >= R) {
                const uint32_t wpr = Wv / R;
                cl_on = my_wave < wpr * R;
                cl_r = my_wave % R;
                cl_rstep = R;
                cl_b = my_wave / R;
                cl_bstep = wpr;
            } else {
                cl_on = my_wave < R;
                cl_r = my_wave;
                cl_rstep = Wv;
            }
            if (cl_on) {
                cl_n = a.clist_cnt[cl_r];
                if (Wv >= R) {
                    const uint32_t per_wave = (cl_n + cl_bstep - 1u) / cl_bstep;
                    const uint32_t lo = (uint32_t)a.clist_min_batch;
                    cl_bs = per_wave >= 64u ? 64u : (per_wave < lo ? lo : per_wave);
                }
            }
        }
    }
    if constexpr (FUSED && !SAMPLED)
        apm_stage_image(reinterpret_cast<uint4 *>(smem), sv->bitmap, 2048, tid, THREADS);
    apm_stage_image(reinterpret_cast<uint4 *>(s_img), a.image, a.image_len >> 4, tid, THREADS);
    for (int i = tid; i < a.n_pats; i += THREADS) s_cnt[i] = 0u;
    __syncthreads();

    const __amdgpu_buffer_rsrc_t rs =
        __builtin_amdgcn_make_buffer_rsrc(const_cast<uint8_t *>(a.text), 0, (int)(uint32_t)a.avail_pad, 0x00020000);
    const uint32_t avail = (uint32_t)a.avail;
    const uint32_t cs = (uint32_t)a.code_shift;

    ApmVerifyCore<BAND> core{a, rs, avail, s_kext, s_masks, s_pat, s_cnt, lane, reinterpret_cast<const uint32_t *>(s_img + a.o_kinfo),
                             reinterpret_cast<const uint2 *>(s_img + a.o_pinfo)};
    typedef ApmWin Win;
    auto load_win = [&](uint32_t a0, Win &o) __attribute__((always_inline)) { core.load_global(a0, o); };

    uint32_t n_surv = 0;
    uint32_t item_lo = 0;
    constexpr uint32_t STEP = SAMPLED ? 8u : 2u;
    const bool listed = n_listed < (uint32_t)a.n_mask_blocks / 4u || (!FUSED && a.clist != nullptr);
    const uint32_t NB = FUSED ? (uint32_t)((sv->nchunks + 3) >> 2) : (listed ? n_listed : (uint32_t)a.n_mask_blocks);
    const uint32_t n_waves_launch = (uint32_t)(FUSED ? sv->n_main_blocks : (int)gridDim.x) * (uint32_t)(THREADS / 64);
    const uint32_t ch_fit = NB / (4u * n_waves_launch);
    const uint32_t CH = SAMPLED ? APM_WORK_CH8 : (listed ? 1u : (ch_fit >= APM_WORK_CH ? APM_WORK_CH : (ch_fit < 1u ? 1u : ch_fit)));
    const uint32_t NC = (NB + CH - 1u) / CH;
    const uint32_t NG = (uint32_t)a.work_groups, grp = (my_wave ^ (my_wave >> 5)) % NG;
    const uint32_t f_g = (uint32_t)(((uint64_t)NC * grp) / NG), n_g = (uint32_t)(((uint64_t)NC * (grp + 1u)) / NG) - f_g;
    uint32_t *const ctr = a.work + ((uint32_t)a.work_epoch & 1u) * (APM_WORK_GROUPS * APM_WORK_STRIDE) + grp * APM_WORK_STRIDE;
    if (blockIdx.x == 0 && tid < APM_WORK_GROUPS) a.work[(((uint32_t)a.work_epoch + 1u) & 1u) * (APM_WORK_GROUPS * APM_WORK_STRIDE) + (uint32_t)tid * APM_WORK_STRIDE] = 0u;
    auto grab = [&]() __attribute__((always_inline)) -> uint32_t {
        return lane == 0 ? __hip_atomic_fetch_add(ctr, 1u, __ATOMIC_RELAXED, __HIP_MEMORY_SCOPE_AGENT) : 0u;
    };
    uint32_t grab_v = grab();
    uint32_t it_b = 0, it_end = 0;
    bool it_done = false;
    constexpr bool STATIC_BLOCKS = FUSED && SAMPLED;
    const uint32_t n_waves_all = (uint32_t)(FUSED ? sv->n_main_blocks : (int)gridDim.x) * (uint32_t)(THREADS / 64);
    uint32_t st_b = my_wave;
    auto it_next = [&](uint32_t &b) __attribute__((always_inline)) -> bool {
        if constexpr (STATIC_BLOCKS) {
            if (st_b >= NB) return false;
            b = st_b;
            st_b += n_waves_all;
            return true;
        }
        if (it_b >= it_end) {
            if (it_done) return false;
            const uint32_t i = (uint32_t)__builtin_amdgcn_readfirstlane((int)grab_v);
            if (i >= n_g) { it_done = true; return false; }
            it_b = (f_g + i) * CH;
            it_end = it_b + CH < NB ? it_b + CH : NB;
            grab_v = grab();
        }
        b = it_b++;
        return true;
    };
    constexpr int AHEAD = FUSED ? 1 : (SAMPLED ? 4 : APM_VERIFY_AHEAD);
    constexpr uint32_t NONE = 0xffffffffu;
    uint32_t hm = 0, hm_q[AHEAD], hb_q[AHEAD];
    if constexpr (!FUSED) {
#pragma unroll
        for (int i = 0; i < AHEAD; ++i) {
            uint32_t b = NONE;
            hb_q[i] = it_next(b) ? (listed ? a.blist[b] : b) : NONE;
            hm_q[i] = hb_q[i] != NONE ? a.masks[(uint64_t)hb_q[i] * 64 + (uint64_t)lane] : 0u;
        }
    }
#ifdef APM_MEASURE
    if (APM_SKIP(a, 512) && lane == 0 && my_wave < APM_STATS_WAVES) a.stats[8 + 2 * my_wave] = wall_clock64();
#endif
    uint32_t blk = 0;
    uint32_t qcount = 0;
    const uint32_t nch32 = FUSED ? (uint32_t)sv->nchunks : 0u;
    const uint32_t tile0 = FUSED ? (uint32_t)sv->tile0 : 0u;
    constexpr bool PREF = FUSED && SAMPLED;
    u32x4 pf_r[4];
    uint32_t pf_sl[4];
    uint32_t pf_b = 0xffffffffu;
    bool pf_started = false;
    auto pf_issue = [&](uint32_t b) __attribute__((always_inline)) {
        const uint32_t g = tile0 + b * 4096u + 16u * (uint32_t)lane;
#pragma unroll
        for (int j = 0; j < 4; ++j) pf_r[j] = __builtin_amdgcn_raw_buffer_load_b128(rs, (int)(g + 1024u * j), 0, 0);
    };
    auto sieve_block = [&](uint32_t b0, uint32_t fb) __attribute__((always_inline)) -> uint32_t {
        const uint32_t g = b0 + 16u * (uint32_t)lane, c0 = fb * 4u;
        uint32_t out = 0;
        if constexpr (SAMPLED) {
            uint32_t sl[4];
#pragma unroll
            for (int j = 0; j < 4; ++j) sl[j] = pf_sl[j];
#pragma unroll
            for (int j = 0; j < 4; ++j) {
                const uint32_t slo = sl[j];
                const uint32_t w0 = s_bmp[slo & 2047u], w1 = s_bmp[(slo >> 16) & 2047u];
                const uint32_t h = ((w0 >> ((slo >> 11) & 31u)) & 1u) | (((w1 >> (slo >> 27)) & 1u) << 1);
                out |= (c0 + j < nch32 ? h : 0u) << (8 * j);
            }
            {
                uint32_t pend = out, cur = 0, curbit = 0, slo_c = 0, tsel = 0;
                bool act = false;
                for (;;) {
                    if (!act && pend) {
                        curbit = (uint32_t)__builtin_ctz(pend);
                        pend &= pend - 1u;
                        tsel = curbit & 1u;
                        const uint32_t j = curbit >> 3;
#pragma unroll
                        for (int q = 0; q < 4; ++q)
                            if (j == (uint32_t)q) slo_c = sl[q];
                        cur = keys.first(tsel ? (slo_c >> 16) : (slo_c & 0xffffu));
                        act = true;
                    }
                    if (!__builtin_amdgcn_ballot_w64(act)) break;
                    if (act && a.o_rc) {
                        const uint32_t kid = ApmKeyList::kid(cur, 11u), rr = ApmKeyList::r(cur, 11u);
                        const uint2 rc = reinterpret_cast<const uint2 *>(s_img + a.o_rc)[(kid * 8u + rr) * 2u + tsel];
                        if (((rc.x ^ slo_c) & rc.y) == 0u) act = false;
                        else if (ApmKeyList::last(cur)) { act = false; out &= ~(1u << curbit); }
                        else cur = keys.next(cur);
                    } else if (act) {
                        const uint32_t kid = ApmKeyList::kid(cur, 11u), rr = ApmKeyList::r(cur, 11u);
                        const uint32_t kx = s_kext[kid];
                        const int at = (int)(kx & 0xffffu), len = (int)((kx >> 16) & 0xffu);
                        const int sh8 = (int)(8u * tsel) - (int)rr;
                        uint32_t B[4];
                        apm_lds_dwords<4>(s_pat, at - sh8, B);
                        const uint32_t pc = apm_pack4(B[0], cs) | (apm_pack4(B[1], cs) << 8) | (apm_pack4(B[2], cs) << 16) | (apm_pack4(B[3], cs) << 24);
                        const int i0 = sh8 > 0 ? sh8 : 0, i1 = len + sh8 < 16 ? len + sh8 : 16;
                        const uint32_t mhi = i1 >= 16 ? 0xffffffffu : ((1u << (2 * i1)) - 1u), mlo = (1u << (2 * i0)) - 1u;
                        if ((((pc ^ slo_c) & mhi) & ~mlo) == 0u) act = false;
                        else if (ApmKeyList::last(cur)) { act = false; out &= ~(1u << curbit); }
                        else cur = keys.next(cur);
                    }
                }
            }
        } else {
            u32x4 r[4];
#pragma unroll
            for (int j = 0; j < 4; ++j) r[j] = __builtin_amdgcn_raw_buffer_load_b128(rs, (int)(g + 1024u * j), 0, 0);
            const v2u32 tl = __builtin_amdgcn_raw_buffer_load_b64(rs, (int)(b0 + 4096u), 0, 0);
            uint32_t slo[5];
#pragma unroll
            for (int j = 0; j < 4; ++j) slo[j] = apm_pack16(r[j].x, r[j].y, r[j].z, r[j].w, cs);
            slo[4] = apm_pack4(tl.x, cs) | (apm_pack4(tl.y, cs) << 8);
#pragma unroll
            for (int j = 0; j < 4; ++j) {
                const uint32_t hits = apm_lookup2_chunk(slo[j], (uint32_t)__builtin_amdgcn_readfirstlane((int)slo[j + 1]));
                out |= (c0 + j < nch32 ? hits >> 24 : 0u) << (8 * j);
                __builtin_amdgcn_sched_barrier(0);
            }
        }
        return out;
    };
    auto next_cand = [&](uint32_t &q, bool &hv) __attribute__((always_inline)) -> bool {
        if constexpr (!FUSED && !SAMPLED) {
            while (cl_on) {
                const uint32_t o = cl_b * cl_bs;
                if (o < cl_n) {
                    const uint32_t nb = cl_n - o < cl_bs ? cl_n - o : cl_bs;
                    hv = (uint32_t)lane < nb;
                    q = hv ? a.clist[(size_t)cl_r * a.clist_cap + o + (uint32_t)lane] : 0u;
                    cl_b += cl_bstep;
                    return true;
                }
                cl_r += cl_rstep;
                cl_b = 0;
                if (cl_r >= (uint32_t)a.clist_regions) { cl_on = false; break; }
                cl_n = a.clist_cnt[cl_r];
            }
        }
        while (qcount < 64u) {
            if (!__builtin_amdgcn_ballot_w64(hm != 0u)) {
                if constexpr (FUSED) {
                    uint32_t b;
                    if constexpr (PREF) {
                        if (!pf_started) {
                            pf_started = true;
                            uint32_t nb;
                            if (it_next(nb)) { pf_b = nb; pf_issue(nb); }
                        }
                        if (pf_b == 0xffffffffu) break;
                        b = pf_b;
#pragma unroll
                        for (int j = 0; j < 4; ++j) pf_sl[j] = apm_pack16(pf_r[j].x, pf_r[j].y, pf_r[j].z, pf_r[j].w, cs);
                        uint32_t nb;
                        if (it_next(nb)) { pf_b = nb; pf_issue(nb); }
                        else pf_b = 0xffffffffu;
                    } else if (!it_next(b)) break;
                    blk = tile0 + b * 4096u;
                    hm = sieve_block(blk, b);
                    continue;
                }
                if (hb_q[0] == NONE) break;
                blk = (uint32_t)(a.tile0 + (int64_t)hb_q[0] * 4096);
                hm = hm_q[0];
#pragma unroll
                for (int i = 0; i + 1 < AHEAD; ++i) { hm_q[i] = hm_q[i + 1]; hb_q[i] = hb_q[i + 1]; }
                {
                    uint32_t b = NONE;
                    hb_q[AHEAD - 1] = it_next(b) ? (listed ? a.blist[b] : b) : NONE;
                    hm_q[AHEAD - 1] = hb_q[AHEAD - 1] != NONE ? a.masks[(uint64_t)hb_q[AHEAD - 1] * 64 + (uint64_t)lane] : 0u;
                }
                continue;
            }
            const bool has = hm != 0u;
            const uint32_t t = has ? (uint32_t)__builtin_ctz(hm) : 0u;
            hm &= hm - 1u;
            apm_wave_append(s_q, qcount, has, (blk + (t >> 3) * 1024u + 16u * (uint32_t)lane + (SAMPLED ? (t & 1u) * 8u : (t & 7u) * 2u)) / STEP);
        }
        q = 0;
        hv = false;
        if (qcount == 0u) return false;
        const uint32_t nb = qcount < 64u ? qcount : 64u;
        hv = (uint32_t)lane < nb;
        if (hv) q = s_q[lane];
        if (qcount > 64u) {
            const uint32_t rest = s_q[64 + lane];
            if ((uint32_t)lane < qcount - 64u) s_q[lane] = rest;
        }
        qcount -= nb;
        return true;
    };
    bool done = false, active = false, have = false;
    uint32_t p = 0, str = 0, s = 0, pend = 0;
    uint32_t cur = 0;
    Win win, win_n, wk;
    constexpr uint32_t PSH = SAMPLED ? 3u : 1u;
    constexpr uint32_t KBITS = SAMPLED ? 11u : 15u;
    uint32_t q_n = 0;
    bool have_n = false;
    bool ex_n = true;
    constexpr int PIPE = FUSED ? APM_FUSED_PIPE : APM_VERIFY_PIPE;
    uint32_t q_nn = 0;
    bool have_nn = false, ex_nn = true;
    load_win(0u, win_n);
    for (;;) {
        if (n_surv * NSH - item_lo >= 64u || (done && n_surv)) {
            const uint32_t avail_items = n_surv * NSH - item_lo, proc = done ? avail_items : (avail_items & ~63u);
            for (uint32_t w0 = 0; w0 < proc; w0 += 64) {
                const uint32_t wi = item_lo + w0 + (uint32_t)lane;
                const bool live = w0 + (uint32_t)lane < proc;
                const uint2 e = live ? s_surv[wi / NSH] : make_uint2(0u, 0u);
                const int dl = (int)(wi % NSH) - BAND;
                uint32_t wpat = 0, wj = 0, word = 0;
                bool hit = live && core.dp_match(e.y, e.x, dl, wpat, wj, word);
#ifdef APM_MEASURE
                if (APM_SKIP(a, 64)) hit = false;
#endif
                core.template count_matches<APM_DEDUP_WIDE(BAND, SAMPLED, FUSED), APM_DEDUP_PREFETCH(BAND, SAMPLED, FUSED)>(hit, wpat, wj, word);
            }
            const uint32_t s_first = (item_lo + proc) / NSH, left = n_surv - s_first;
            const uint2 keep = (uint32_t)lane < left ? s_surv[s_first + (uint32_t)lane] : make_uint2(0u, 0u);
            if ((uint32_t)lane < left) s_surv[lane] = keep;
            item_lo = item_lo + proc - s_first * NSH;
            n_surv = left;
        }
        if (done) break;
        if (!active && pend) {
            const uint32_t par = (pend & 1u) ? 0u : 1u;
            pend &= pend - 1u;
            cur = keys.first((str >> (2u * par)) & 0xffffu);
            s = p + par;
            active = true;
            if constexpr (SAMPLED) {
                s = p - ApmKeyList::r(cur, KBITS);
                if (s > p) s = 0xffffffffu;
                load_win(s & ~3u, wk);
            }
        }
        if (!__builtin_amdgcn_ballot_w64(active)) {
            if (!ex_n) { done = true; continue; }
            p = q_n << PSH;
            have = have_n;
            win = win_n;
            if constexpr (PIPE == 2) {
                ex_n = ex_nn;
                q_n = q_nn;
                have_n = have_nn;
                load_win((q_n << PSH) & ~3u, win_n);
                ex_nn = next_cand(q_nn, have_nn);
            } else {
                ex_n = next_cand(q_n, have_n);
                load_win((q_n << PSH) & ~3u, win_n);
            }
            str = 0;
#pragma unroll
            for (int i = 0; i < 3; ++i) {
                const uint32_t b4 = __builtin_amdgcn_alignbyte(win.w[i + 1], win.w[i], p & 3u);
                str |= apm_pack4(b4, cs) << (8 * i);
            }
            const uint32_t x0 = str & 0xffffu, x1 = (str >> 2) & 0xffffu;
            pend = have ? (((s_bmp[x0 & 2047u] >> (x0 >> 11)) & 1u) | (SAMPLED ? 0u : (((s_bmp[x1 & 2047u] >> (x1 >> 11)) & 1u) << 1))) : 0u;
#ifdef APM_MEASURE
            if (APM_SKIP(a, 8)) pend = 0;
#endif
            continue;
        }
        bool ok = false;
        if (active) ok = core.stage1(ApmKeyList::kid(cur, KBITS), s, SAMPLED ? wk : win, load_win);
#ifdef APM_MEASURE
        if (APM_SKIP(a, 16)) ok = false;
#endif
        const unsigned long long mask = __builtin_amdgcn_ballot_w64(ok);
#ifdef APM_MEASURE
        if (APM_SKIP(a, 256) && mask && lane == 0) atomicAdd(&a.stats[1], (unsigned long long)__builtin_popcountll(mask));
#endif
        if (mask) {
            const uint32_t idx = n_surv + apm_wave_rank(mask);
            if (ok) s_surv[idx] = make_uint2(s, ApmKeyList::kid(cur, KBITS));
            n_surv += (uint32_t)__builtin_popcountll(mask);
        }
        if (active) {
            if (ApmKeyList::last(cur)) active = false;
            else {
                cur = keys.next(cur);
                if constexpr (SAMPLED) {
                    s = p - ApmKeyList::r(cur, KBITS);
                    if (s > p) s = 0xffffffffu;
                    load_win(s & ~3u, wk);
                }
            }
        }
    }

#ifdef APM_MEASURE
    if (APM_SKIP(a, 512) && lane == 0 && my_wave < APM_STATS_WAVES) a.stats[9 + 2 * my_wave] = wall_clock64();
#endif
    __syncthreads();
    for (int i = tid; i < a.n_pats; i += THREADS) {
        const uint32_t cnt = s_cnt[i];
        if (cnt) atomicAdd(&a.counts[a.pats[i].index], (unsigned long long)cnt);
    }
}

template <int BAND, int THREADS, bool SAMPLED>
__global__ __launch_bounds__(THREADS, (BAND == 1 && THREADS == 256 && !SAMPLED) ? 6 : 4) void apm_verify_kernel(ApmVerifyArgs a) {
    extern __shared__ __attribute__((aligned(16))) uint8_t smem[];
    apm_verify_body<BAND, THREADS, SAMPLED, false>(a, nullptr, smem);
}

static size_t apm_verify_lds_bytes_t(const ApmVerifyArgs &a, int threads) {
    return (size_t)a.image_len + (size_t)((a.n_pats + 3) & ~3) * 4 + (size_t)(threads / 64) * ((size_t)apm_verify_scap(a.band) * 8 + 128 * 4) +
           16;
}

template <typename Family>
static const void *apm_band_fn(int band, const Family &k) {
    switch (band) {
    case 0: return k.template fn<0>();
    case 1: return k.template fn<1>();
    case 2: return k.template fn<2>();
    case 3: return k.template fn<3>();
    default: return nullptr;
    }
}
struct ApmVerifyFamily {
    int threads, stride;
    template <int BAND>
    const void *fn() const {
        if (threads == 512) return stride == 8 ? (const void *)apm_verify_kernel<BAND, 512, true> : (const void *)apm_verify_kernel<BAND, 512, false>;
        return stride == 8 ? (const void *)apm_verify_kernel<BAND, 256, true> : (const void *)apm_verify_kernel<BAND, 256, false>;
    }
};
static const void *apm_verify_fn(int band, int threads, int stride) { return apm_band_fn(band, ApmVerifyFamily{threads, stride}); }

int apm_verify_geometry(const ApmVerifyArgs &a, int *threads) {
    const int blocks = apm_best_geometry([&](int t) { return apm_verify_fn(a.band, t, a.stride); }, 256, 512, 256,
                                         [&](int t) { return apm_verify_lds_bytes_t(a, t); }, 8, 0, threads);
    if (blocks) return blocks;
    *threads = 256;
    return 2;
}

hipError_t apm_launch_verify(const ApmVerifyArgs &a, int threads, int max_blocks, int *work_epoch, hipStream_t s) {
    if (a.n_pats <= 0) return hipSuccess;
    const void *fn = apm_verify_fn(a.band, threads, a.stride);
    if (!fn) return hipErrorInvalidValue;
    ApmVerifyArgs args = a;
    args.n_blocks = max_blocks < 1 ? 1 : max_blocks;
#ifdef APM_MEASURE
    if (const char *e = getenv("APM_VERIFY_GRID_PCT")) args.n_blocks = std::max(1, (int)((long)args.n_blocks * atoi(e) / 100));
    if (const char *e = getenv("APM_MEASURE_SKIP")) args.skip_mask = atoi(e);
#endif
    args.work_groups = std::min<long>(APM_WORK_GROUPS, (long)args.n_blocks * (threads / 64));
    args.work_epoch = *work_epoch;
    void *kargs[] = {&args};
    const hipError_t e = hipLaunchKernel(fn, dim3((unsigned)args.n_blocks), dim3((unsigned)threads), kargs, apm_verify_lds_bytes_t(a, threads), s);
    if (e == hipSuccess) ++*work_epoch;
    return e;
}

template <int BAND, bool SAMPLED>
__global__ __launch_bounds__(APM_FUSED_MAX_THREADS, SAMPLED ? (BAND == 0 ? 7 : (BAND == 1 ? APM_FUSED_S_WAVES : 5)) : (BAND == 0 ? 6 : 5)) void apm_fused_kernel(ApmFusedArgs f) {
    extern __shared__ __attribute__((aligned(16))) uint8_t smem[];
    if ((int)blockIdx.x >= f.s.n_main_blocks) {
        apm_tail_body(f.s.tail, (int)blockIdx.x - f.s.n_main_blocks, reinterpret_cast<uint4 *>(smem), (int)threadIdx.x);
        return;
    }
    apm_verify_body<BAND, 0, SAMPLED, true>(f.v, &f.s, smem);
}

struct ApmFusedFamily {
    int stride;
    template <int BAND>
    const void *fn() const { return stride == 8 ? (const void *)apm_fused_kernel<BAND, true> : (const void *)apm_fused_kernel<BAND, false>; }
};
static const void *apm_fused_fn(int band, int stride) { return apm_band_fn(band, ApmFusedFamily{stride}); }

size_t apm_fused_lds_bytes(const ApmFusedArgs &a, int threads) {
    const size_t need = (a.s.stride == 8 ? 0 : 32768) + apm_verify_lds_bytes_t(a.v, threads);
    return need < 4096 + 256 ? 4096 + 256 : need;
}

int apm_fused_geometry(const ApmFusedArgs &a, int *threads) {
    const void *fn = apm_fused_fn(a.v.band, a.s.stride);
    *threads = 0;
    if (!fn) return 0;
    apm_ensure_max_lds(fn);
#ifdef APM_MEASURE
    static const int forced = getenv("APM_FUSED_THREADS") ? atoi(getenv("APM_FUSED_THREADS")) : 0;
#else
    constexpr int forced = 0;
#endif
    return apm_best_geometry([&](int) { return fn; }, APM_FUSED_MAX_THREADS, 256, -64, [&](int t) { return apm_fused_lds_bytes(a, t); }, INT_MAX, forced, threads);
}

hipError_t apm_launch_fused(const ApmFusedArgs &a, int threads, int max_blocks, int *work_epoch, hipStream_t s) {
    if (a.s.nchunks <= 0 || a.v.n_pats <= 0) return hipSuccess;
    const void *fn = apm_fused_fn(a.v.band, a.s.stride);
    if (!fn || threads < 64 || threads > APM_FUSED_MAX_THREADS || (threads & 63)) return hipErrorInvalidValue;
    const size_t lds = apm_fused_lds_bytes(a, threads);
    const int64_t n_fb = (a.s.nchunks + 3) / 4, want = (n_fb + threads / 64 - 1) / (threads / 64);
    const int64_t nb = want < max_blocks ? want : (max_blocks < 1 ? 1 : max_blocks);
    ApmFusedArgs args = a;
    args.s.n_main_blocks = (int)nb;
    args.v.n_blocks = (int)nb;
#ifdef APM_MEASURE
    if (const char *e = getenv("APM_MEASURE_SKIP")) args.v.skip_mask = atoi(e);
#endif
    if (lds > 48 * 1024) apm_ensure_max_lds(fn);
    args.v.work_groups = (int)std::min<int64_t>(APM_WORK_GROUPS, nb * (threads / 64));
    args.v.work_epoch = *work_epoch;
    void *kargs[] = {&args};
    const hipError_t e = hipLaunchKernel(fn, dim3((unsigned)(nb + a.s.n_tail)), dim3((unsigned)threads), kargs, lds, s);
    if (e == hipSuccess) ++*work_epoch;
    return e;
}
```

Baseline: 799800000 billion.

## Add latency-hiding verify kernel variant for band-1 candidate lists

Adds a LAT variant of the verify kernel, built in its own translation unit, for band 1, stride 1, 256 threads with candidate lists. It prefetches the first candidate window before staging the LDS image and loads the next 16-byte text block ahead inside the banded DP. It also checks bytes 16-31 of exact segments as one vector compare and stages partner-extension text into per-lane LDS. Whole blocks with no candidate entries exit early. The cost is extra LDS per wave, which can lower occupancy, and more code paths, in exchange for less global-load latency on the critical path.

```diff
diff --git a/inf560-approximate-pattern-matching_amd/csrc/apm_device.h b/inf560-approximate-pattern-matching_amd/csrc/apm_device.h
--- a/inf560-approximate-pattern-matching_amd/csrc/apm_device.h
+++ b/inf560-approximate-pattern-matching_amd/csrc/apm_device.h
@@ -39,9 +39,16 @@
     for (int i = 0; i < N; ++i) out[i] = __builtin_amdgcn_alignbyte(w[i + 1], w[i], sh);
 }
 
+template <typename Text, typename = void>
+struct ApmTextAhead { static constexpr bool value = false; };
+template <typename Text>
+struct ApmTextAhead<Text, decltype((void)Text::kAhead)> { static constexpr bool value = Text::kAhead; };
+
 template <int BAND, typename Text>
 __device__ __forceinline__ bool apm_banded_verify(const Text &tx, const uint8_t *pb, int poff, int m, int k) {
     const uint8_t *p = pb + poff;
+    constexpr bool kAhead = ApmTextAhead<Text>::value;
+    (void)kAhead;
     if constexpr (BAND == 0 && Text::kBlocks) {
         int mism = 0;
         for (int xb = 0; xb < m; xb += 16) {
@@ -74,7 +81,12 @@
         int x0 = 1;
         if (m >= 16 && tx.can16(m)) {
             uint32_t T[4], P[5];
+            uint32_t Tn[4] = {0u, 0u, 0u, 0u};
+            (void)Tn;
             tx.load16(T);
+            if constexpr (kAhead && Text::kBlocks) {
+                if (m > 16) tx.load16_at(16, Tn);
+            }
             apm_lds_dwords<5>(pb, poff, P);
 #pragma unroll
             for (int x = 1; x <= 16; ++x) {
@@ -104,7 +116,13 @@
             if constexpr (Text::kBlocks) {
                 for (int xb = 17; xb <= m; xb += 16) {
                     uint32_t Tb[4], Pb[6];
-                    tx.load16_at(xb - 1, Tb);
+                    if constexpr (kAhead) {
+#pragma unroll
+                        for (int i = 0; i < 4; ++i) Tb[i] = Tn[i];
+                        if (xb + 16 <= m) tx.load16_at(xb + 15, Tn);
+                    } else {
+                        tx.load16_at(xb - 1, Tb);
+                    }
                     apm_lds_dwords<6>(pb, poff + xb - 1 - BAND, Pb);
 #pragma unroll
                     for (int xi = 0; xi < 16; ++xi) {
diff --git a/inf560-approximate-pattern-matching_amd/csrc/apm_rec.h b/inf560-approximate-pattern-matching_amd/csrc/apm_rec.h
--- a/inf560-approximate-pattern-matching_amd/csrc/apm_rec.h
+++ b/inf560-approximate-pattern-matching_amd/csrc/apm_rec.h
@@ -18,6 +18,8 @@
 #define apm_sieve2cfdg_kernel apm_sieve2cfdg_kernel_rec
 #define apm_sieve8_kernel apm_sieve8_kernel_rec
 #define apm_verify_kernel apm_verify_kernel_rec
+#define apm_verify_lat_kernel apm_verify_lat_kernel_rec
+#define apm_verify_lat_fn apm_verify_lat_fn_rec
 #define apm_fused_kernel apm_fused_kernel_rec
 #define apm_launch_bitpar apm_launch_bitpar_rec
 #define apm_launch_bitpar_wide apm_launch_bitpar_wide_rec
diff --git a/inf560-approximate-pattern-matching_amd/csrc/apm_scan.hip b/inf560-approximate-pattern-matching_amd/csrc/apm_scan.hip
--- a/inf560-approximate-pattern-matching_amd/csrc/apm_scan.hip
+++ b/inf560-approximate-pattern-matching_amd/csrc/apm_scan.hip
@@ -72,6 +72,7 @@
     int clist_region_cap = env_1_to_64("APM_CLIST_REGION_CAP", 0);
     int clist_min_batch = env_1_to_64("APM_CLIST_MIN_BATCH", 8);
     int clist_pools = std::max(0, env_int("APM_CLIST_POOLS", 8));
+    int verify_lat = env_int("APM_VERIFY_LAT", -1);
     int cf_dp_diag = env_int("APM_CF_DP_DIAG", 1);
     int filter_dma = env_int("APM_FILTER_DMA", 1);
     int filter_stream = env_int("APM_FILTER_STREAM", 1);
@@ -352,7 +353,17 @@
 #endif
     va.work = ds.d_work;
     if (!D.blocks_per_cu) D.blocks_per_cu = apm_verify_geometry(va, &D.threads);
-    APM_LAUNCH(ctx, ds, "verify", APM_PICK(g, apm_launch_verify)(va, D.threads, ds.n_cu * D.blocks_per_cu, &ds.work_epoch, ds.stream));
+    const int lat_env = scan_env().verify_lat;
+    bool lat = va.clist != nullptr && va.band == 1 && va.stride == 1 && D.threads == 256 && (lat_env < 0 ? r.clist_pools > 0 : lat_env != 0);
+    if (lat && !D.lat_threads) {
+        va.lat = 1;
+        D.lat_blocks_per_cu = apm_verify_geometry(va, &D.lat_threads);
+        if (D.lat_blocks_per_cu < 1) D.lat_threads = -1;
+    }
+    lat = lat && D.lat_threads == 256;
+    va.lat = lat ? 1 : 0;
+    ds.last_verify_lat = va.lat;
+    APM_LAUNCH(ctx, ds, "verify", APM_PICK(g, apm_launch_verify)(va, lat ? D.lat_threads : D.threads, ds.n_cu * (lat ? D.lat_blocks_per_cu : D.blocks_per_cu), &ds.work_epoch, ds.stream));
     return APM_OK;
 }
 
@@ -612,7 +623,7 @@
     rc = run_tiled_launches(ctx, ds, g, tails, fused_run || sieve_run);
     if (rc) return rc;
     ds.last_fused = fused_run;
-    if (!sieve_run) { ds.last_mask_blocks = 0; ds.last_clist_regions = 0; ds.last_clist_pools = 0; ds.last_sieve_waves = 0; ds.last_cf_dp_form = 0; }
+    if (!sieve_run) { ds.last_mask_blocks = 0; ds.last_clist_regions = 0; ds.last_clist_pools = 0; ds.last_sieve_waves = 0; ds.last_cf_dp_form = 0; ds.last_verify_lat = 0; }
     rc = launch_generic_group(ctx, ds, g, plan.longs, ds.d_long_descs, 2);
     if (rc) return rc;
     if (ctx->timing_on) HIP_TRY(ctx, hipEventRecord(ds.ev_mstop, ds.stream));
diff --git a/inf560-approximate-pattern-matching_amd/csrc/apm_sieve.h b/inf560-approximate-pattern-matching_amd/csrc/apm_sieve.h
--- a/inf560-approximate-pattern-matching_amd/csrc/apm_sieve.h
+++ b/inf560-approximate-pattern-matching_amd/csrc/apm_sieve.h
@@ -70,6 +70,7 @@
     uint32_t clist_cap;
     int clist_regions;
     int clist_min_batch;
+    int lat;
     int64_t tile0;
     int64_t n_mask_blocks;
     int n_blocks;
diff --git a/inf560-approximate-pattern-matching_amd/csrc/apm_state.h b/inf560-approximate-pattern-matching_amd/csrc/apm_state.h
--- a/inf560-approximate-pattern-matching_amd/csrc/apm_state.h
+++ b/inf560-approximate-pattern-matching_amd/csrc/apm_state.h
@@ -19,6 +19,7 @@
     uint32_t *d_pinfo = nullptr;
     uint32_t *d_kpart = nullptr;
     int blocks_per_cu = 0, threads = 256;
+    int lat_blocks_per_cu = 0, lat_threads = 0;
     int fused_blocks_per_cu = 0, fused_threads = 0;
     int cf_threads = 0, cf_blocks_per_cu = 0;
 };
@@ -119,6 +120,7 @@
     int pool_epoch = 0;
     int pool_dirty[2] = {0, 0};
     int last_clist_pools = 0;
+    int last_verify_lat = 0;
     unsigned long long *d_stats = nullptr;
     int last_sieve_waves = 0;
     int last_cf_dp_form = 0;
diff --git a/inf560-approximate-pattern-matching_amd/csrc/apm_stats.hip b/inf560-approximate-pattern-matching_amd/csrc/apm_stats.hip
--- a/inf560-approximate-pattern-matching_amd/csrc/apm_stats.hip
+++ b/inf560-approximate-pattern-matching_amd/csrc/apm_stats.hip
@@ -115,6 +115,7 @@
     if (n == "sieve_stride") { *value = S.on ? (double)S.stride : 0.0; return APM_OK; }
     if (n == "sieve_clist") { *value = ds.last_clist_regions ? 1.0 : 0.0; return APM_OK; }
     if (n == "sieve_clist_pools") { *value = (double)ds.last_clist_pools; return APM_OK; }
+    if (n == "verify_lat") { *value = (double)ds.last_verify_lat; return APM_OK; }
     if (n == "sieve_waves") { *value = (double)ds.last_sieve_waves; return APM_OK; }
     if (n == "sieve_mask_bytes") {
         *value = (double)ds.last_mask_blocks * 256.0;
diff --git a/inf560-approximate-pattern-matching_amd/csrc/apm_verify.hip b/inf560-approximate-pattern-matching_amd/csrc/apm_verify.hip
--- a/inf560-approximate-pattern-matching_amd/csrc/apm_verify.hip
+++ b/inf560-approximate-pattern-matching_amd/csrc/apm_verify.hip
@@ -46,9 +46,18 @@
     __device__ __forceinline__ int byte(int x) const { return (int)__builtin_amdgcn_raw_buffer_load_b8(rs, (int)(off + (uint32_t)x), 0, 0); }
 };
 
+struct ApmBufTextAhead : ApmBufText {
+    static constexpr bool kAhead = true;
+};
+
 struct ApmWin { uint32_t w[6]; };
-
-template <int BAND>
+__device__ __forceinline__ void apm_load_win(__amdgpu_buffer_rsrc_t rs, uint32_t a0, ApmWin &o) {
+    const u32x4 lo = __builtin_amdgcn_raw_buffer_load_b128(rs, (int)a0, 0, 0);
+    const v2u32 hi = __builtin_amdgcn_raw_buffer_load_b64(rs, (int)(a0 + 16u), 0, 0);
+    o.w[0] = lo.x; o.w[1] = lo.y; o.w[2] = lo.z; o.w[3] = lo.w; o.w[4] = hi.x; o.w[5] = hi.y;
+}
+
+template <int BAND, bool LAT = false>
 struct ApmVerifyCore {
     static constexpr int NSH = 2 * BAND + 1;
     static constexpr bool PAIRS = BAND >= 1;
@@ -62,12 +71,9 @@
     int lane;
     const uint32_t *s_kinfo;
     const uint2 *s_pinfo;
-
-    __device__ __forceinline__ void load_global(uint32_t a0, ApmWin &o) const {
-        const u32x4 lo = __builtin_amdgcn_raw_buffer_load_b128(rs, (int)a0, 0, 0);
-        const v2u32 hi = __builtin_amdgcn_raw_buffer_load_b64(rs, (int)(a0 + 16u), 0, 0);
-        o.w[0] = lo.x; o.w[1] = lo.y; o.w[2] = lo.z; o.w[3] = lo.w; o.w[4] = hi.x; o.w[5] = hi.y;
-    }
+    uint8_t *s_pt = nullptr;
+
+    __device__ __forceinline__ void load_global(uint32_t a0, ApmWin &o) const { apm_load_win(rs, a0, o); }
     __device__ __forceinline__ int gbyte(uint32_t pos) const {
         return (int)__builtin_amdgcn_raw_buffer_load_b8(rs, (int)pos, 0, 0);
     }
@@ -85,14 +91,47 @@
         apm_lds_dwords<4>(s_pat, at, B);
         const uint4 mk = s_masks[len < 16 ? len : 16];
         if ((((A[0] ^ B[0]) & mk.x) | ((A[1] ^ B[1]) & mk.y) | ((A[2] ^ B[2]) & mk.z) | ((A[3] ^ B[3]) & mk.w)) != 0u) return false;
-        for (int x = 16; x < len; ++x)
-            if (gbyte(s + (uint32_t)x) != (int)s_pat[at + x]) return false;
+        if constexpr (LAT) {
+            if (len > 16) {
+                uint32_t A2[4], B2[4];
+                ApmBufText{rs, s + 16u}.load16(A2);
+                apm_lds_dwords<4>(s_pat, at + 16, B2);
+                const uint4 mk2 = s_masks[len < 32 ? len - 16 : 16];
+                if ((((A2[0] ^ B2[0]) & mk2.x) | ((A2[1] ^ B2[1]) & mk2.y) | ((A2[2] ^ B2[2]) & mk2.z) | ((A2[3] ^ B2[3]) & mk2.w)) != 0u) return false;
+            }
+            for (int x = 32; x < len; ++x)
+                if (gbyte(s + (uint32_t)x) != (int)s_pat[at + x]) return false;
+        } else {
+            for (int x = 16; x < len; ++x)
+                if (gbyte(s + (uint32_t)x) != (int)s_pat[at + x]) return false;
+        }
         if (!PAIRS || side == 0) return true;
         if (n == 31) {
             const uint32_t kp = a.kpart[kid];
             const int poff = (int)(s_pinfo[s_kinfo[kid] & 0xfffu].x & 0xffffu), ap = (int)(kp & 0xffffu), nn = (int)(kp >> 16), ap1 = ap + nn;
             const bool fwd = side == 1;
-            auto T = [&](int i) { return fwd ? gbyte(s + (uint32_t)len + (uint32_t)i) : gbyte(s - 1u - (uint32_t)i); };
+            bool staged = false;
+            uint32_t pt0 = 0;
+            const uint8_t *pt = nullptr;
+            if constexpr (LAT) {
+                if (nn <= 47) {
+                    staged = true;
+                    pt0 = (fwd ? s + (uint32_t)len : s - 1u - (uint32_t)nn) & ~3u;
+                    uint32_t *const ptw = reinterpret_cast<uint32_t *>(s_pt) + lane * 13;
+                    uint32_t w[13];
+#pragma unroll
+                    for (int d = 0; d < 13; ++d) w[d] = __builtin_amdgcn_raw_buffer_load_b32(rs, (int)(pt0 + 4u * (uint32_t)d), 0, 0);
+#pragma unroll
+                    for (int d = 0; d < 13; ++d) ptw[d] = w[d];
+                    pt = reinterpret_cast<const uint8_t *>(ptw);
+                }
+            }
+            auto T = [&](int i) {
+                if constexpr (LAT) {
+                    if (staged) return (int)pt[(fwd ? s + (uint32_t)len + (uint32_t)i : s - 1u - (uint32_t)i) - pt0];
+                }
+                return fwd ? gbyte(s + (uint32_t)len + (uint32_t)i) : gbyte(s - 1u - (uint32_t)i);
+            };
             auto P = [&](int i) { return fwd ? (int)s_pat[poff + ap + i] : (int)s_pat[poff + ap1 - 1 - i]; };
             int i = 0;
             while (i < nn && T(i) == P(i)) ++i;
@@ -168,7 +207,8 @@
 #ifdef APM_MEASURE
         if (APM_SKIP(a, 256)) atomicAdd(&a.stats[2], 1ull);
 #endif
-        return apm_banded_verify<BAND>(ApmBufText{rs, (uint32_t)j}, s_pat, poff, m, a.k);
+        if constexpr (LAT) return apm_banded_verify<BAND>(ApmBufTextAhead{{rs, (uint32_t)j}}, s_pat, poff, m, a.k);
+        else return apm_banded_verify<BAND>(ApmBufText{rs, (uint32_t)j}, s_pat, poff, m, a.k);
     }
 
     template <bool PREF>
@@ -179,19 +219,21 @@
         if (o < 0) return false;
         ApmWin w2;
         load_global((uint32_t)o & ~3u, w2);
-        if constexpr (PAIRS && PREF) {
-            const uint32_t kx = s_kext[kid];
-            const uint32_t len = (kx >> 16) & 0xffu, side = kx >> 29;
-            const bool ask = side != 0u && ((kx >> 24) & 31u) != 31u && (side == 1u ? len != 0u : o >= 20);
-            const uint32_t pa = ask ? (side == 1u ? (uint32_t)o + len : (uint32_t)o - 20u) & ~3u : 0xffffff00u;
-            ApmWin wp;
-            load_global(pa, wp);
-            return stage1(kid, (uint32_t)o, w2, [&](uint32_t a0, ApmWin &o2) {
-                if (a0 == pa) o2 = wp;
-                else load_global(a0, o2);
-            });
-        }
+        if constexpr (PAIRS && PREF) return stage1_partner_ahead(kid, o, w2);
         return stage1(kid, (uint32_t)o, w2, [&](uint32_t a0, ApmWin &o2) { load_global(a0, o2); });
+    }
+
+    __device__ __forceinline__ bool stage1_partner_ahead(uint32_t kid, int64_t o, const ApmWin &win) const {
+        const uint32_t kx = s_kext[kid];
+        const uint32_t len = (kx >> 16) & 0xffu, side = kx >> 29;
+        const bool ask = side != 0u && ((kx >> 24) & 31u) != 31u && (side == 1u ? len != 0u : o >= 20);
+        const uint32_t pa = ask ? (side == 1u ? (uint32_t)o + len : (uint32_t)o - 20u) & ~3u : 0xffffff00u;
+        ApmWin wp;
+        load_global(pa, wp);
+        return stage1(kid, (uint32_t)o, win, [&](uint32_t a0, ApmWin &o2) {
+            if (a0 == pa) o2 = wp;
+            else load_global(a0, o2);
+        });
     }
 
     template <bool WIDE, bool PREF>
@@ -264,9 +306,10 @@
 
 };
 
+#define APM_VERIFY_PT_BYTES 52
 __host__ __device__ constexpr int apm_verify_scap(int band) { return ((64 + 2 * band) / (2 * band + 1) + 63 + 7) & ~7; }
 
-template <int BAND, int THREADS_T, bool SAMPLED, bool FUSED>
+template <int BAND, int THREADS_T, bool SAMPLED, bool FUSED, bool LAT = false>
 __device__ __forceinline__ void apm_verify_body(const ApmVerifyArgs &a, const ApmSieve2Args *sv, uint8_t *smem) {
     const int THREADS = THREADS_T ? THREADS_T : (int)blockDim.x;
     const int tid = threadIdx.x, lane = tid & 63;
@@ -292,9 +335,26 @@
     const uint32_t n_listed = (!FUSED && a.blist != nullptr) ? *a.blist_ctr : 0xffffffffu;
     bool cl_on = false;
     uint32_t cl_r = 0, cl_rstep = 0, cl_b = 0, cl_bstep = 1, cl_n = 0, cl_bs = 64;
+    bool wg_entries = true;
+    (void)wg_entries;
     if constexpr (!FUSED && !SAMPLED) {
         if (a.clist) {
             const uint32_t R = (uint32_t)a.clist_regions, Wv = (uint32_t)gridDim.x * (uint32_t)(THREADS / 64);
+            if constexpr (LAT) {
+                if (Wv >= R) {
+                    const uint32_t wpr = Wv / R;
+                    wg_entries = false;
+#pragma unroll
+                    for (int w = 0; w < THREADS / 64; ++w) {
+                        const uint32_t ow = blockIdx.x * (uint32_t)(THREADS / 64) + (uint32_t)w;
+                        if (ow < wpr * R) {
+                            const uint32_t n = a.clist_cnt[ow % R], per_wave = (n + wpr - 1u) / wpr, lo = (uint32_t)a.clist_min_batch;
+                            const uint32_t bs = per_wave >= 64u ? 64u : (per_wave < lo ? lo : per_wave);
+                            wg_entries = wg_entries || (ow / R) * bs < n;
+                        }
+                    }
+                }
+            }
             if (Wv >= R) {
                 const uint32_t wpr = Wv / R;
                 cl_on = my_wave < wpr * R;
@@ -317,6 +377,28 @@
             }
         }
     }
+    typedef ApmWin Win;
+    const bool lat_no_rows = LAT && a.clist != nullptr && n_listed == 0u;
+    uint32_t q_first = 0;
+    bool have_first = false;
+    Win win_first;
+    if constexpr (LAT) {
+        if (blockIdx.x == 0 && tid < APM_WORK_GROUPS) a.work[(((uint32_t)a.work_epoch + 1u) & 1u) * (APM_WORK_GROUPS * APM_WORK_STRIDE) + (uint32_t)tid * APM_WORK_STRIDE] = 0u;
+        if (lat_no_rows && !wg_entries) {
+#ifdef APM_MEASURE
+            if (APM_SKIP(a, 512) && lane == 0 && my_wave < APM_STATS_WAVES) a.stats[8 + 2 * my_wave] = a.stats[9 + 2 * my_wave] = wall_clock64();
+#endif
+            return;
+        }
+        if (cl_on && cl_b * cl_bs < cl_n) {
+            const uint32_t o = cl_b * cl_bs, nb = cl_n - o < cl_bs ? cl_n - o : cl_bs;
+            have_first = (uint32_t)lane < nb;
+            q_first = have_first ? a.clist[(size_t)cl_r * a.clist_cap + o + (uint32_t)lane] : 0u;
+            cl_b += cl_bstep;
+        }
+        apm_load_win(__builtin_amdgcn_make_buffer_rsrc(const_cast<uint8_t *>(a.text), 0, (int)(uint32_t)a.avail_pad, 0x00020000),
+                     (q_first << 1) & ~3u, win_first);
+    }
     if constexpr (FUSED && !SAMPLED)
         apm_stage_image(reinterpret_cast<uint4 *>(smem), sv->bitmap, 2048, tid, THREADS);
     apm_stage_image(reinterpret_cast<uint4 *>(s_img), a.image, a.image_len >> 4, tid, THREADS);
@@ -328,9 +410,10 @@
     const uint32_t avail = (uint32_t)a.avail;
     const uint32_t cs = (uint32_t)a.code_shift;
 
-    ApmVerifyCore<BAND> core{a, rs, avail, s_kext, s_masks, s_pat, s_cnt, lane, reinterpret_cast<const uint32_t *>(s_img + a.o_kinfo),
-                             reinterpret_cast<const uint2 *>(s_img + a.o_pinfo)};
-    typedef ApmWin Win;
+    ApmVerifyCore<BAND, LAT> core{a, rs, avail, s_kext, s_masks, s_pat, s_cnt, lane, reinterpret_cast<const uint32_t *>(s_img + a.o_kinfo),
+                                  reinterpret_cast<const uint2 *>(s_img + a.o_pinfo)};
+    if constexpr (LAT)
+        core.s_pt = reinterpret_cast<uint8_t *>(s_q - wv * 128 + (THREADS / 64) * 128) + wv * (64 * APM_VERIFY_PT_BYTES);
     auto load_win = [&](uint32_t a0, Win &o) __attribute__((always_inline)) { core.load_global(a0, o); };
 
     uint32_t n_surv = 0;
@@ -345,13 +428,15 @@
     const uint32_t NG = (uint32_t)a.work_groups, grp = (my_wave ^ (my_wave >> 5)) % NG;
     const uint32_t f_g = (uint32_t)(((uint64_t)NC * grp) / NG), n_g = (uint32_t)(((uint64_t)NC * (grp + 1u)) / NG) - f_g;
     uint32_t *const ctr = a.work + ((uint32_t)a.work_epoch & 1u) * (APM_WORK_GROUPS * APM_WORK_STRIDE) + grp * APM_WORK_STRIDE;
-    if (blockIdx.x == 0 && tid < APM_WORK_GROUPS) a.work[(((uint32_t)a.work_epoch + 1u) & 1u) * (APM_WORK_GROUPS * APM_WORK_STRIDE) + (uint32_t)tid * APM_WORK_STRIDE] = 0u;
+    if constexpr (!LAT)
+        if (blockIdx.x == 0 && tid < APM_WORK_GROUPS) a.work[(((uint32_t)a.work_epoch + 1u) & 1u) * (APM_WORK_GROUPS * APM_WORK_STRIDE) + (uint32_t)tid * APM_WORK_STRIDE] = 0u;
     auto grab = [&]() __attribute__((always_inline)) -> uint32_t {
         return lane == 0 ? __hip_atomic_fetch_add(ctr, 1u, __ATOMIC_RELAXED, __HIP_MEMORY_SCOPE_AGENT) : 0u;
     };
-    uint32_t grab_v = grab();
+    uint32_t grab_v = 0;
+    if (!lat_no_rows) grab_v = grab();
     uint32_t it_b = 0, it_end = 0;
-    bool it_done = false;
+    bool it_done = lat_no_rows;
     constexpr bool STATIC_BLOCKS = FUSED && SAMPLED;
     const uint32_t n_waves_all = (uint32_t)(FUSED ? sv->n_main_blocks : (int)gridDim.x) * (uint32_t)(THREADS / 64);
     uint32_t st_b = my_wave;
@@ -552,7 +637,13 @@
     constexpr int PIPE = FUSED ? APM_FUSED_PIPE : APM_VERIFY_PIPE;
     uint32_t q_nn = 0;
     bool have_nn = false, ex_nn = true;
-    load_win(0u, win_n);
+    if constexpr (LAT) {
+        q_n = q_first;
+        have_n = have_first;
+        win_n = win_first;
+    } else {
+        load_win(0u, win_n);
+    }
     for (;;) {
         if (n_surv * NSH - item_lo >= 64u || (done && n_surv)) {
             const uint32_t avail_items = n_surv * NSH - item_lo, proc = done ? avail_items : (avail_items & ~63u);
@@ -616,7 +707,11 @@
             continue;
         }
         bool ok = false;
-        if (active) ok = core.stage1(ApmKeyList::kid(cur, KBITS), s, SAMPLED ? wk : win, load_win);
+        if constexpr (LAT) {
+            if (active) ok = core.stage1_partner_ahead(ApmKeyList::kid(cur, KBITS), (int64_t)s, win);
+        } else {
+            if (active) ok = core.stage1(ApmKeyList::kid(cur, KBITS), s, SAMPLED ? wk : win, load_win);
+        }
 #ifdef APM_MEASURE
         if (APM_SKIP(a, 16)) ok = false;
 #endif
@@ -652,6 +747,15 @@
     }
 }
 
+#ifdef APM_VERIFY_LAT_UNIT
+__global__ __launch_bounds__(256, 4) void apm_verify_lat_kernel(ApmVerifyArgs a) {
+    extern __shared__ __attribute__((aligned(16))) uint8_t smem[];
+    apm_verify_body<1, 256, false, false, true>(a, nullptr, smem);
+}
+const void *apm_verify_lat_fn() { return (const void *)apm_verify_lat_kernel; }
+#else
+const void *apm_verify_lat_fn();
+
 template <int BAND, int THREADS, bool SAMPLED>
 __global__ __launch_bounds__(THREADS, (BAND == 1 && THREADS == 256 && !SAMPLED) ? 6 : 4) void apm_verify_kernel(ApmVerifyArgs a) {
     extern __shared__ __attribute__((aligned(16))) uint8_t smem[];
@@ -660,6 +764,7 @@
 
 static size_t apm_verify_lds_bytes_t(const ApmVerifyArgs &a, int threads) {
     return (size_t)a.image_len + (size_t)((a.n_pats + 3) & ~3) * 4 + (size_t)(threads / 64) * ((size_t)apm_verify_scap(a.band) * 8 + 128 * 4) +
+           (a.lat ? (size_t)(threads / 64) * 64 * APM_VERIFY_PT_BYTES : 0) +
            16;
 }
 
@@ -681,10 +786,16 @@
         return stride == 8 ? (const void *)apm_verify_kernel<BAND, 256, true> : (const void *)apm_verify_kernel<BAND, 256, false>;
     }
 };
-static const void *apm_verify_fn(int band, int threads, int stride) { return apm_band_fn(band, ApmVerifyFamily{threads, stride}); }
+static const void *apm_verify_fn(int band, int threads, int stride, bool lat) {
+    if (lat) return (band == 1 && threads == 256 && stride == 1) ? apm_verify_lat_fn() : nullptr;
+    return apm_band_fn(band, ApmVerifyFamily{threads, stride});
+}
 
 int apm_verify_geometry(const ApmVerifyArgs &a, int *threads) {
-    const int blocks = apm_best_geometry([&](int t) { return apm_verify_fn(a.band, t, a.stride); }, 256, 512, 256,
+    if (a.lat && apm_verify_lds_bytes_t(a, 256) > 48 * 1024) { *threads = 0; return 0; }
+    if (a.lat) return apm_best_geometry([&](int t) { return apm_verify_fn(a.band, t, a.stride, true); }, 256, 256, 256,
+                                        [&](int t) { return apm_verify_lds_bytes_t(a, t); }, 8, 0, threads);
+    const int blocks = apm_best_geometry([&](int t) { return apm_verify_fn(a.band, t, a.stride, false); }, 256, 512, 256,
                                          [&](int t) { return apm_verify_lds_bytes_t(a, t); }, 8, 0, threads);
     if (blocks) return blocks;
     *threads = 256;
@@ -693,8 +804,8 @@
 
 hipError_t apm_launch_verify(const ApmVerifyArgs &a, int threads, int max_blocks, int *work_epoch, hipStream_t s) {
     if (a.n_pats <= 0) return hipSuccess;
-    const void *fn = apm_verify_fn(a.band, threads, a.stride);
-    if (!fn) return hipErrorInvalidValue;
+    const void *fn = apm_verify_fn(a.band, threads, a.stride, a.lat != 0);
+    if (!fn || (a.lat && !a.clist)) return hipErrorInvalidValue;
     ApmVerifyArgs args = a;
     args.n_blocks = max_blocks < 1 ? 1 : max_blocks;
 #ifdef APM_MEASURE
@@ -765,3 +876,4 @@
     if (e == hipSuccess) ++*work_epoch;
     return e;
 }
+#endif
diff --git a/inf560-approximate-pattern-matching_amd/csrc/apm_verify_lat.hip b/inf560-approximate-pattern-matching_amd/csrc/apm_verify_lat.hip
--- /dev/null
+++ b/inf560-approximate-pattern-matching_amd/csrc/apm_verify_lat.hip
@@ -0,0 +1,2 @@
+#define APM_VERIFY_LAT_UNIT
+#include "apm_verify.hip"
```

After: 806600000 billion, median of 6. About the same (+0.9%).
